# tum-vision/mem

Measured on AMD Instinct MI355X. Metric: pretrain samples/sec (ViT-B, 224^2 event voxels), higher is better.
Workload: dtype bf16; 1 GPU; MEM pretrain ViT-Base/16, 224^2 2-bin event voxels, bf16, batch 256 per GPU (BASELINE configs[1]); step = rasterize 256x30k events + event_norm + masks + ViT fwd/CE/bwd + clip + AdamW; global_batch=256, parallelism=dp1, stochastic_depth=work skipping, optimizer=AdamW as one launch in front of the next forward, last_block_mlp_rows=rows that reach the head

## Files before the change

### mem_amd/csrc/rowops.hip

```cpp
#include "common.h"
#include "dropout.hpp"

namespace {

using namespace memhip;

typedef __attribute__((ext_vector_type(4))) __bf16 bf16x4;
typedef __attribute__((ext_vector_type(8))) __bf16 bf16x8;

__device__ __forceinline__ float wsum(float v) {
  for (int o = 32; o > 0; o >>= 1) v += __shfl_xor(v, o);
  return v;
}
__device__ __forceinline__ float wmax(float v) {
  for (int o = 32; o > 0; o >>= 1) v = fmaxf(v, __shfl_xor(v, o));
  return v;
}

__device__ __forceinline__ float div_newton(float a, float b, float r) {
  const float q0 = a * r;
  return fmaf(fmaf(-q0, b, a), r, q0);
}

constexpr int kMaxChunks = 8;

__global__ __launch_bounds__(256) void ln_fwd_kernel(const float* __restrict__ x, long long ldx,
                                                     const int* __restrict__ row_idx, int R, int D,
                                                     const float* __restrict__ gamma,
                                                     const float* __restrict__ beta, float eps,
                                                     __bf16* __restrict__ y, long long ldy,
                                                     float* __restrict__ mean, float* __restrict__ rstd) {
  const int lane = threadIdx.x & 63;
  const int r = blockIdx.x * 4 + (threadIdx.x >> 6);
  if (r >= R) return;
  const long long src = row_idx ? row_idx[r] : r;
  const float4* xr = reinterpret_cast<const float4*>(x + src * ldx);
  const int nch = D >> 2;
  float4 v[kMaxChunks];
  float s = 0.f;
#pragma unroll
  for (int c = 0; c < kMaxChunks; ++c) {
    const int i = lane + c * 64;
    if (i < nch) { v[c] = xr[i]; s += (v[c].x + v[c].y) + (v[c].z + v[c].w); }
  }
  const float mu = wsum(s) / (float)D;
  float q = 0.f;
#pragma unroll
  for (int c = 0; c < kMaxChunks; ++c) {
    const int i = lane + c * 64;
    if (i < nch) {
      const float a = v[c].x - mu, b = v[c].y - mu, cc = v[c].z - mu, d = v[c].w - mu;
      q += (a * a + b * b) + (cc * cc + d * d);
    }
  }
  const float var = wsum(q) / (float)D;
  const float rs = 1.0f / sqrtf(var + eps);
  if (lane == 0) { mean[r] = mu; rstd[r] = rs; }
  const float4* g4 = reinterpret_cast<const float4*>(gamma);
  const float4* b4 = reinterpret_cast<const float4*>(beta);
  bf16x4* yr = reinterpret_cast<bf16x4*>(y + (long long)r * ldy);
#pragma unroll
  for (int c = 0; c < kMaxChunks; ++c) {
    const int i = lane + c * 64;
    if (i < nch) {
      const float4 g = g4[i], b = b4[i];
      bf16x4 o;
      o[0] = (__bf16)((v[c].x - mu) * rs * g.x + b.x);
      o[1] = (__bf16)((v[c].y - mu) * rs * g.y + b.y);
      o[2] = (__bf16)((v[c].z - mu) * rs * g.z + b.z);
      o[3] = (__bf16)((v[c].w - mu) * rs * g.w + b.w);
      yr[i] = o;
    }
  }
}


template <int NCH>
__global__ __launch_bounds__(256) void ln_bwd_kernel(const __bf16* __restrict__ dy, long long lddy,
                                                     const float* __restrict__ x, long long ldx,
                                                     const int* __restrict__ row_idx, int R, int D,
                                                     const float* __restrict__ gamma,
                                                     const float* __restrict__ mean,
                                                     const float* __restrict__ rstd,
                                                     float* __restrict__ dres, long long lddres,
                                                     int accumulate, float* __restrict__ dgamma,
                                                     float* __restrict__ dbeta) {
  extern __shared__ float red[];
  const int lane = threadIdx.x & 63, wave = threadIdx.x >> 6;
  const int nch = D >> 2;
  const float4* g4 = reinterpret_cast<const float4*>(gamma);
  float4 ag[NCH], ab[NCH], gm[NCH];
#pragma unroll
  for (int c = 0; c < NCH; ++c) {
    ag[c] = float4{0, 0, 0, 0};
    ab[c] = float4{0, 0, 0, 0};
    gm[c] = (lane + c * 64 < nch) ? g4[lane + c * 64] : float4{0, 0, 0, 0};
  }
  for (int r = blockIdx.x * 4 + wave; r < R; r += gridDim.x * 4) {
    const long long src = row_idx ? row_idx[r] : r;
    const float4* xr = reinterpret_cast<const float4*>(x + src * ldx);
    const bf16x4* dyr = reinterpret_cast<const bf16x4*>(dy + (long long)r * lddy);
    const float mu = mean[r], rs = rstd[r];
    float4 xh[NCH], gg[NCH], prev[NCH];
    float4* o = reinterpret_cast<float4*>(dres + src * lddres);
    if (accumulate) {
#pragma unroll
      for (int c = 0; c < NCH; ++c)
        if (lane + c * 64 < nch) prev[c] = o[lane + c * 64];
    }
    float s1 = 0.f, s2 = 0.f;
#pragma unroll
    for (int c = 0; c < NCH; ++c) {
      const int i = lane + c * 64;
      if (i < nch) {
        const float4 xv = xr[i];
        const bf16x4 d4 = dyr[i];
        const float4 g = gm[c];
        const float d0 = (float)d4[0], d1 = (float)d4[1], d2 = (float)d4[2], d3 = (float)d4[3];
        xh[c] = float4{(xv.x - mu) * rs, (xv.y - mu) * rs, (xv.z - mu) * rs, (xv.w - mu) * rs};
        gg[c] = float4{d0 * g.x, d1 * g.y, d2 * g.z, d3 * g.w};
        s1 += (gg[c].x + gg[c].y) + (gg[c].z + gg[c].w);
        s2 += (gg[c].x * xh[c].x + gg[c].y * xh[c].y) + (gg[c].z * xh[c].z + gg[c].w * xh[c].w);
        ag[c].x += d0 * xh[c].x; ag[c].y += d1 * xh[c].y; ag[c].z += d2 * xh[c].z; ag[c].w += d3 * xh[c].w;
        ab[c].x += d0; ab[c].y += d1; ab[c].z += d2; ab[c].w += d3;
      }
    }
    const float m1 = wsum(s1) / (float)D, m2 = wsum(s2) / (float)D;
#pragma unroll
    for (int c = 0; c < NCH; ++c) {
      const int i = lane + c * 64;
      if (i < nch) {
        float4 d{rs * (gg[c].x - m1 - xh[c].x * m2), rs * (gg[c].y - m1 - xh[c].y * m2),
                 rs * (gg[c].z - m1 - xh[c].z * m2), rs * (gg[c].w - m1 - xh[c].w * m2)};
        if (accumulate) { const float4 p = prev[c]; d.x += p.x; d.y += p.y; d.z += p.z; d.w += p.w; }
        o[i] = d;
      }
    }
  }
  float4* rg = reinterpret_cast<float4*>(red + (size_t)wave * 2 * D);
  float4* rb = reinterpret_cast<float4*>(red + (size_t)wave * 2 * D + D);
#pragma unroll
  for (int c = 0; c < NCH; ++c) {
    const int i = lane + c * 64;
    if (i < nch) { rg[i] = ag[c]; rb[i] = ab[c]; }
  }
  __syncthreads();
  for (int n = threadIdx.x; n < D; n += 256) {
    float a = 0.f, b = 0.f;
#pragma unroll
    for (int w = 0; w < 4; ++w) { a += red[(size_t)w * 2 * D + n]; b += red[(size_t)w * 2 * D + D + n]; }
    atomicAdd(dgamma + n, a);
    atomicAdd(dbeta + n, b);
  }
}

constexpr int kBrMaxChunks = 8;

template <int NCH, class... Drop>
__global__ __launch_bounds__(256) void branch_bwd_kernel(const float* __restrict__ dx, long long lddx,
                                                         const __bf16* __restrict__ y, long long ldy,
                                                         const float* __restrict__ gamma,
                                                         const float* __restrict__ rowmask, float keep,
                                                         int rps, int M, int D, __bf16* __restrict__ dyo,
                                                         long long lddy, float* __restrict__ dgamma,
                                                         float* __restrict__ dbias, const int* __restrict__ out_map,
                                                         Drop... drop) {
  extern __shared__ float red[];
  const int lane = threadIdx.x & 63, wave = threadIdx.x >> 6;
  const int nch = D >> 2;
  float4 g[NCH], ag[NCH], ab[NCH];
  const float rk = __frcp_rn(keep);
#pragma unroll
  for (int c = 0; c < NCH; ++c) {
    const int i = lane + c * 64;
    g[c] = (gamma && i < nch) ? reinterpret_cast<const float4*>(gamma)[i] : float4{1.f, 1.f, 1.f, 1.f};
    ag[c] = float4{0, 0, 0, 0};
    ab[c] = float4{0, 0, 0, 0};
  }
  const int stride = gridDim.x * 4;
  for (int m0 = blockIdx.x * 4 + wave; m0 < M; m0 += 2 * stride) {
    float4 dv[2][NCH];
    bf16x4 yv[2][NCH];
    float kk[2];
    long long mo[2];
#pragma unroll
    for (int u = 0; u < 2; ++u) {
      const int m = m0 + u * stride;
      const int mc = m < M ? m : M - 1;
      const float4* dr = reinterpret_cast<const float4*>(dx + (long long)mc * lddx);
      kk[u] = rowmask ? rowmask[mc / rps] : 1.f;
      mo[u] = m < M ? m : -1;
      if (out_map && m < M) {
        const int smp = mc / rps, co = out_map[smp];
        mo[u] = co < 0 ? -1 : (long long)co * rps + (mc - smp * rps);
      }
      if (mo[u] < 0) continue;
#pragma unroll
      for (int c = 0; c < NCH; ++c) {
        const int i = lane + c * 64;
        if (i < nch) {
          dv[u][c] = dr[i];
          if (y) yv[u][c] = reinterpret_cast<const bf16x4*>(y + (long long)mc * ldy)[i];
        }
      }
    }
#pragma unroll
    for (int u = 0; u < 2; ++u) {
      if (mo[u] < 0) continue;
      bf16x4* orow = reinterpret_cast<bf16x4*>(dyo + mo[u] * lddy);
      const float k = kk[u];
#pragma unroll
      for (int c = 0; c < NCH; ++c) {
        const int i = lane + c * 64;
        if (i < nch) {
          float4 d = dv[u][c];
          if (rowmask || out_map) {
            d.x = div_newton(d.x * k, keep, rk); d.y = div_newton(d.y * k, keep, rk);
            d.z = div_newton(d.z * k, keep, rk); d.w = div_newton(d.w * k, keep, rk);
          }
          if constexpr (sizeof...(Drop) > 0) {
            const DropParams dp = (drop, ...);
            const unsigned kb = dropout_keep8(dp, (unsigned)(dp.row0 + m0 + u * stride), (unsigned)(i >> 1)) >> ((i & 1) * 4);
            d.x = __fmul_rn(d.x, dropout_mul(dp, kb, 0)); d.y = __fmul_rn(d.y, dropout_mul(dp, kb, 1));
            d.z = __fmul_rn(d.z, dropout_mul(dp, kb, 2)); d.w = __fmul_rn(d.w, dropout_mul(dp, kb, 3));
          }
          if (y) {
            const bf16x4 yy = yv[u][c];
            ag[c].x += d.x * (float)yy[0]; ag[c].y += d.y * (float)yy[1];
            ag[c].z += d.z * (float)yy[2]; ag[c].w += d.w * (float)yy[3];
          }
          bf16x4 o;
          o[0] = (__bf16)(d.x * g[c].x); o[1] = (__bf16)(d.y * g[c].y);
          o[2] = (__bf16)(d.z * g[c].z); o[3] = (__bf16)(d.w * g[c].w);
          orow[i] = o;
          ab[c].x += (float)o[0]; ab[c].y += (float)o[1]; ab[c].z += (float)o[2]; ab[c].w += (float)o[3];
        }
      }
    }
  }
  float4* rg = reinterpret_cast<float4*>(red + (size_t)wave * 2 * D);
  float4* rb = reinterpret_cast<float4*>(red + (size_t)wave * 2 * D + D);
#pragma unroll
  for (int c = 0; c < NCH; ++c) {
    const int i = lane + c * 64;
    if (i < nch) { rg[i] = ag[c]; rb[i] = ab[c]; }
  }
  __syncthreads();
  for (int n = threadIdx.x; n < D; n += 256) {
    float a = 0.f, b = 0.f;
#pragma unroll
    for (int w = 0; w < 4; ++w) { a += red[(size_t)w * 2 * D + n]; b += red[(size_t)w * 2 * D + D + n]; }
    if (dgamma) atomicAdd(dgamma + n, a);
    if (dbias) atomicAdd(dbias + n, b);
  }
}

template <int NCH, bool HAS_Y, class... Drop>
__global__ __launch_bounds__(256) void ln_bwd_branch_kernel(const __bf16* __restrict__ dy, long long lddy,
                                                            const float* __restrict__ x, long long ldx, int R, int D,
                                                            const float* __restrict__ gamma,
                                                            const float* __restrict__ mean, const float* __restrict__ rstd,
                                                            float* __restrict__ dres, long long lddres,
                                                            float* __restrict__ dgamma, float* __restrict__ dbeta,
                                                            const __bf16* __restrict__ yb, long long ldyb,
                                                            const float* __restrict__ gb, const float* __restrict__ rowmask,
                                                            float keep, int rps, __bf16* __restrict__ dyo, long long lddyo,
                                                            float* __restrict__ dgb, float* __restrict__ dbiasb,
                                                            const int* __restrict__ in_map, const int* __restrict__ out_map,
                                                            Drop... drop) {
  extern __shared__ float red[];
  const int lane = threadIdx.x & 63, wave = threadIdx.x >> 6;
  const int nch = D >> 2;
  float4 ag[NCH], ab[NCH], bg[HAS_Y ? NCH : 1], bb[NCH];
  const float4* g4 = reinterpret_cast<const float4*>(gamma);
  const float4* gb4 = reinterpret_cast<const float4*>(gb);
  const float rk = __frcp_rn(keep);
#pragma unroll
  for (int c = 0; c < NCH; ++c) {
    ag[c] = ab[c] = bb[c] = float4{0, 0, 0, 0};
    if (HAS_Y) bg[c] = float4{0, 0, 0, 0};
  }
  const int rstride = gridDim.x * 4;
  float4 xn[NCH], pn[NCH];
  bf16x4 dn[NCH], yn[HAS_Y ? NCH : 1];
  long long rin_n = 0, rout_n = 0;
  auto load_row = [&](int r) {
    rin_n = r; rout_n = r;
    if (in_map || out_map) {
      const int smp = r / rps, off = r - smp * rps;
      if (in_map) { const int ci = in_map[smp]; rin_n = ci < 0 ? -1 : (long long)ci * rps + off; }
      if (out_map) { const int co = out_map[smp]; rout_n = co < 0 ? -1 : (long long)co * rps + off; }
    }
    if (rin_n < 0 && rout_n < 0) return;
    const float4* xr = reinterpret_cast<const float4*>(x + (long long)r * ldx);
    const bf16x4* dyr = reinterpret_cast<const bf16x4*>(dy + (rin_n < 0 ? 0 : rin_n) * lddy);
    const float4* o = reinterpret_cast<const float4*>(dres + (long long)r * lddres);
#pragma unroll
    for (int c = 0; c < NCH; ++c) {
      const int i = lane + c * 64;
      if (i < nch) {
        pn[c] = o[i];
        if (rin_n >= 0) {
          xn[c] = xr[i];
          dn[c] = dyr[i];
        }
        if constexpr (HAS_Y) yn[c] = reinterpret_cast<const bf16x4*>(yb + (long long)r * ldyb)[i];
      }
    }
  };
  int r = blockIdx.x * 4 + wave;
  if (r < R) load_row(r);
  for (; r < R; r += rstride) {
    const long long rin = rin_n, rout = rout_n;
    if (rin < 0 && rout < 0) {
      if (r + rstride < R) load_row(r + rstride);
      continue;
    }
    float4* o = reinterpret_cast<float4*>(dres + (long long)r * lddres);
    const float mu = rin >= 0 ? mean[rin] : 0.f, rs = rin >= 0 ? rstd[rin] : 0.f;
    const float km = rowmask ? rowmask[r / rps] : 1.f;
    float4 xh[NCH], gg[NCH], prev[NCH];
    bf16x4 yv[HAS_Y ? NCH : 1];
    float s1 = 0.f, s2 = 0.f;
#pragma unroll
    for (int c = 0; c < NCH; ++c) {
      const int i = lane + c * 64;
      if (i < nch) {
        prev[c] = pn[c];
        if constexpr (HAS_Y) yv[c] = yn[c];
        if (rin < 0) {
          xh[c] = gg[c] = float4{0.f, 0.f, 0.f, 0.f};
          continue;
        }
        const float4 xv = xn[c];
        const bf16x4 d4 = dn[c];
        const float d0 = (float)d4[0], d1 = (float)d4[1], d2 = (float)d4[2], d3 = (float)d4[3];
        xh[c] = float4{(xv.x - mu) * rs, (xv.y - mu) * rs, (xv.z - mu) * rs, (xv.w - mu) * rs};
        const float4 gmc = g4[i];
        gg[c] = float4{d0 * gmc.x, d1 * gmc.y, d2 * gmc.z, d3 * gmc.w};
        s1 += (gg[c].x + gg[c].y) + (gg[c].z + gg[c].w);
        s2 += (gg[c].x * xh[c].x + gg[c].y * xh[c].y) + (gg[c].z * xh[c].z + gg[c].w * xh[c].w);
        ag[c].x += d0 * xh[c].x; ag[c].y += d1 * xh[c].y; ag[c].z += d2 * xh[c].z; ag[c].w += d3 * xh[c].w;
        ab[c].x += d0; ab[c].y += d1; ab[c].z += d2; ab[c].w += d3;
      }
    }
    if (r + rstride < R) load_row(r + rstride);
    const float m1 = wsum(s1) / (float)D, m2 = wsum(s2) / (float)D;
    bf16x4* orow = reinterpret_cast<bf16x4*>(dyo + (rout < 0 ? 0 : rout) * lddyo);
#pragma unroll
    for (int c = 0; c < NCH; ++c) {
      const int i = lane + c * 64;
      if (i < nch) {
        float4 d{prev[c].x + rs * (gg[c].x - m1 - xh[c].x * m2), prev[c].y + rs * (gg[c].y - m1 - xh[c].y * m2),
                 prev[c].z + rs * (gg[c].z - m1 - xh[c].z * m2), prev[c].w + rs * (gg[c].w - m1 - xh[c].w * m2)};
        if (rin >= 0) o[i] = d;
        if (rout < 0) continue;
        if (rowmask || out_map) {
          d.x = div_newton(d.x * km, keep, rk); d.y = div_newton(d.y * km, keep, rk);
          d.z = div_newton(d.z * km, keep, rk); d.w = div_newton(d.w * km, keep, rk);
        }
        if constexpr (sizeof...(Drop) > 0) {
          const DropParams dp = (drop, ...);
          const unsigned kb = dropout_keep8(dp, (unsigned)(dp.row0 + r), (unsigned)(i >> 1)) >> ((i & 1) * 4);
          d.x = __fmul_rn(d.x, dropout_mul(dp, kb, 0)); d.y = __fmul_rn(d.y, dropout_mul(dp, kb, 1));
          d.z = __fmul_rn(d.z, dropout_mul(dp, kb, 2)); d.w = __fmul_rn(d.w, dropout_mul(dp, kb, 3));
        }
        if constexpr (HAS_Y) {
          bg[c].x += d.x * (float)yv[c][0]; bg[c].y += d.y * (float)yv[c][1];
          bg[c].z += d.z * (float)yv[c][2]; bg[c].w += d.w * (float)yv[c][3];
        }
        const float4 gbc = gb ? gb4[i] : float4{1.f, 1.f, 1.f, 1.f};
        bf16x4 q;
        q[0] = (__bf16)(d.x * gbc.x); q[1] = (__bf16)(d.y * gbc.y);
        q[2] = (__bf16)(d.z * gbc.z); q[3] = (__bf16)(d.w * gbc.w);
        orow[i] = q;
        bb[c].x += (float)q[0]; bb[c].y += (float)q[1]; bb[c].z += (float)q[2]; bb[c].w += (float)q[3];
      }
    }
  }
  float4* r0 = reinterpret_cast<float4*>(red + (size_t)wave * 4 * D);
#pragma unroll
  for (int c = 0; c < NCH; ++c) {
    const int i = lane + c * 64;
    if (i < nch) { r0[i] = ag[c]; r0[nch + i] = ab[c]; r0[2 * nch + i] = HAS_Y ? bg[HAS_Y ? c : 0] : float4{0, 0, 0, 0}; r0[3 * nch + i] = bb[c]; }
  }
  __syncthreads();
  for (int n = threadIdx.x; n < D; n += 256) {
    float a = 0.f, b = 0.f, c2 = 0.f, d2 = 0.f;
#pragma unroll
    for (int w = 0; w < 4; ++w) {
      const float* rw = red + (size_t)w * 4 * D;
      a += rw[n]; b += rw[D + n]; c2 += rw[2 * D + n]; d2 += rw[3 * D + n];
    }
    atomicAdd(dgamma + n, a);
    atomicAdd(dbeta + n, b);
    if (dgb) atomicAdd(dgb + n, c2);
    if (dbiasb) atomicAdd(dbiasb + n, d2);
  }
}


__global__ __launch_bounds__(256) void layerscale_grad_kernel(const __bf16* __restrict__ W, long long ldw,
                                                              const float* __restrict__ dW, long long lddw,
                                                              const float* __restrict__ b, const float* __restrict__ db,
                                                              const float* __restrict__ gamma, int N, int K,
                                                              float* __restrict__ dgamma) {
  __shared__ float red[4][4];
  const int lane = threadIdx.x & 63, wave = threadIdx.x >> 6;
  const int n0 = blockIdx.x * 4;
  float s[4] = {0.f, 0.f, 0.f, 0.f};
  for (int k0 = 0; k0 < K; k0 += 4096) {
#pragma unroll
    for (int c = 0; c < 4; ++c) {
      const int n = n0 + c < N ? n0 + c : N - 1;
      const __bf16* wr = W + (long long)n * ldw;
      const float* gr = dW + (long long)n * lddw;
#pragma unroll
      for (int u = 0; u < 4; ++u) {
        const int k = k0 + u * 1024 + (int)threadIdx.x * 4;
        if (k < K) {
          const bf16x4 w = *reinterpret_cast<const bf16x4*>(wr + k);
          const float4 g = *reinterpret_cast<const float4*>(gr + k);
          s[c] += (float)w[0] * g.x + (float)w[1] * g.y + (float)w[2] * g.z + (float)w[3] * g.w;
        }
      }
    }
  }
#pragma unroll
  for (int c = 0; c < 4; ++c) {
    const float t = wsum(s[c]);
    if (lane == 0) red[wave][c] = t;
  }
  __syncthreads();
  if (threadIdx.x < 4 && n0 + (int)threadIdx.x < N) {
    const int n = n0 + threadIdx.x;
    float t = (red[0][threadIdx.x] + red[1][threadIdx.x]) + (red[2][threadIdx.x] + red[3][threadIdx.x]);
    if (b && db) t += b[n] * db[n];
    const float g = gamma[n];
    dgamma[n] = g != 0.f ? t / g : 0.f;
  }
}

__global__ __launch_bounds__(256) void embed_bwd_kernel(const float* __restrict__ dx, long long lddx,
                                                        const unsigned char* __restrict__ mask, int B,
                                                        int L, int D, __bf16* __restrict__ dy,
                                                        long long lddy, float* __restrict__ dcls,
                                                        float* __restrict__ dmask) {
  constexpr int U = 7;
  for (int c = threadIdx.x * 4; c < D; c += 256 * 4) {
    float4 cls{0, 0, 0, 0}, am{0, 0, 0, 0};
    for (int b = blockIdx.x; b < B; b += gridDim.x) {
      const float* row0 = dx + (long long)b * (L + 1) * lddx + c;
      const float4 dc = *reinterpret_cast<const float4*>(row0);
      cls.x += dc.x; cls.y += dc.y; cls.z += dc.z; cls.w += dc.w;
      const unsigned char* mk = mask + (long long)b * L;
      __bf16* out = dy + (long long)b * L * lddy + c;
      int p = 0;
      for (; p + U <= L; p += U) {
        float4 d[U];
#pragma unroll
        for (int u = 0; u < U; ++u) d[u] = *reinterpret_cast<const float4*>(row0 + (long long)(1 + p + u) * lddx);
#pragma unroll
        for (int u = 0; u < U; ++u) {
          const float w = (float)mk[p + u], q = 1.0f - w;
          am.x += d[u].x * w; am.y += d[u].y * w; am.z += d[u].z * w; am.w += d[u].w * w;
          bf16x4 o;
          o[0] = (__bf16)(d[u].x * q); o[1] = (__bf16)(d[u].y * q); o[2] = (__bf16)(d[u].z * q); o[3] = (__bf16)(d[u].w * q);
          *reinterpret_cast<bf16x4*>(out + (long long)(p + u) * lddy) = o;
        }
      }
      for (; p < L; ++p) {
        const float4 d = *reinterpret_cast<const float4*>(row0 + (long long)(1 + p) * lddx);
        const float w = (float)mk[p], q = 1.0f - w;
        am.x += d.x * w; am.y += d.y * w; am.z += d.z * w; am.w += d.w * w;
        bf16x4 o;
        o[0] = (__bf16)(d.x * q); o[1] = (__bf16)(d.y * q); o[2] = (__bf16)(d.z * q); o[3] = (__bf16)(d.w * q);
        *reinterpret_cast<bf16x4*>(out + (long long)p * lddy) = o;
      }
    }
    atomicAdd(dcls + c, cls.x); atomicAdd(dcls + c + 1, cls.y);
    atomicAdd(dcls + c + 2, cls.z); atomicAdd(dcls + c + 3, cls.w);
    atomicAdd(dmask + c, am.x); atomicAdd(dmask + c + 1, am.y);
    atomicAdd(dmask + c + 2, am.z); atomicAdd(dmask + c + 3, am.w);
  }
}

template <int VPT>
__global__ __launch_bounds__(256) void ce_kernel(__bf16* __restrict__ logits, long long ld,
                                                 const long long* __restrict__ labels, int V,
                                                 float grad_scale, float* __restrict__ row_loss,
                                                 int* __restrict__ row_correct, int write_grad) {
  __shared__ float sm[4];
  __shared__ int si[4];
  __shared__ float bc[2];
  const int r = blockIdx.x, tid = threadIdx.x, lane = tid & 63, wave = tid >> 6;
  bf16x8* row = reinterpret_cast<bf16x8*>(logits + (long long)r * ld);
  const int nch = V >> 3;
  float v[VPT][8];
  float mx = -INFINITY;
  int amax = 0x7fffffff;
#pragma unroll
  for (int c = 0; c < VPT; ++c) {
    const int i = tid + c * 256;
    if (i < nch) {
      const bf16x8 t = row[i];
#pragma unroll
      for (int k = 0; k < 8; ++k) {
        v[c][k] = (float)t[k];
        if (v[c][k] > mx) { mx = v[c][k]; amax = i * 8 + k; }
      }
    }
  }
  for (int o = 32; o > 0; o >>= 1) {
    const float om = __shfl_xor(mx, o);
    const int oi = __shfl_xor(amax, o);
    if (om > mx || (om == mx && oi < amax)) { mx = om; amax = oi; }
  }
  if (lane == 0) { sm[wave] = mx; si[wave] = amax; }
  __syncthreads();
  if (tid == 0) {
    float m = sm[0]; int a = si[0];
    for (int w = 1; w < 4; ++w) if (sm[w] > m || (sm[w] == m && si[w] < a)) { m = sm[w]; a = si[w]; }
    bc[0] = m; si[0] = a;
  }
  __syncthreads();
  mx = bc[0];
  amax = si[0];
  float s = 0.f;
#pragma unroll
  for (int c = 0; c < VPT; ++c) {
    const int i = tid + c * 256;
    if (i < nch) {
#pragma unroll
      for (int k = 0; k < 8; ++k) { v[c][k] = __expf(v[c][k] - mx); s += v[c][k]; }
    }
  }
  s = wsum(s);
  __syncthreads();
  if (lane == 0) sm[wave] = s;
  __syncthreads();
  if (tid == 0) bc[1] = (sm[0] + sm[1]) + (sm[2] + sm[3]);
  __syncthreads();
  const float sum = bc[1];
  const long long lab = labels[r];
  if (tid == 0) {
    const bool lab_ok = lab >= 0 && lab < V;
    const float zl = lab_ok ? (float)logits[(long long)r * ld + lab] : __builtin_nanf("");
    row_loss[r] = (mx + __logf(sum)) - zl;
    row_correct[r] = (amax == (int)lab) ? 1 : 0;
  }
  if (write_grad) {
    const float inv = 1.0f / sum;
    __syncthreads();
#pragma unroll
    for (int c = 0; c < VPT; ++c) {
      const int i = tid + c * 256;
      if (i < nch) {
        bf16x8 o;
#pragma unroll
        for (int k = 0; k < 8; ++k) {
          float p = v[c][k] * inv;
          if ((long long)(i * 8 + k) == lab) p -= 1.0f;
          o[k] = (__bf16)(p * grad_scale);
        }
        row[i] = o;
      }
    }
  }
}

__global__ __launch_bounds__(256) void ce_reduce_kernel(const float* __restrict__ row_loss,
                                                        const int* __restrict__ row_correct, int M,
                                                        float* __restrict__ out) {
  __shared__ double sd[4];
  __shared__ int sc[4];
  double s = 0.0;
  int c = 0;
  for (int i = threadIdx.x; i < M; i += 256) { s += (double)row_loss[i]; c += row_correct[i]; }
  for (int o = 32; o > 0; o >>= 1) { s += __shfl_xor(s, o); c += __shfl_xor(c, o); }
  if ((threadIdx.x & 63) == 0) { sd[threadIdx.x >> 6] = s; sc[threadIdx.x >> 6] = c; }
  __syncthreads();
  if (threadIdx.x == 0) {
    const double t = (sd[0] + sd[1]) + (sd[2] + sd[3]);
    const int k = sc[0] + sc[1] + sc[2] + sc[3];
    out[0] = (float)(t / (double)M);
    out[1] = (float)k / (float)M;
  }
}

}

extern "C" int memhip_layernorm_fwd(const float* x, int64_t ldx, const int32_t* row_idx, int R, int D,
                                    const float* gamma, const float* beta, float eps, void* y,
                                    int64_t ldy, float* mean, float* rstd, memhip_stream_t stream) {
  MEMHIP_REQUIRE(R >= 0 && D > 0 && D % 4 == 0 && D <= 64 * 4 * kMaxChunks, "layernorm_fwd: bad R=%d D=%d", R, D);
  if (R == 0) return MEMHIP_OK;
  MEMHIP_REQUIRE(x && gamma && beta && y && mean && rstd, "layernorm_fwd: null pointer");
  MEMHIP_REQUIRE(ldx % 4 == 0 && ldy % 4 == 0, "layernorm_fwd: ld must be a multiple of 4");
  hipLaunchKernelGGL(ln_fwd_kernel, dim3(cdiv(R, 4)), dim3(256), 0, as_stream(stream), x, (long long)ldx,
                     row_idx, R, D, gamma, beta, eps, (__bf16*)y, (long long)ldy, mean, rstd);
  return check_launch("layernorm_fwd");
}

extern "C" int memhip_layernorm_bwd(const void* dy, int64_t lddy, const float* x, int64_t ldx,
                                    const int32_t* row_idx, int R, int D, const float* gamma,
                                    const float* mean, const float* rstd, float* dres, int64_t lddres,
                                    int accumulate, float* dgamma, float* dbeta, memhip_stream_t stream) {
  MEMHIP_REQUIRE(R >= 0 && D > 0 && D % 4 == 0 && D <= 64 * 4 * kMaxChunks, "layernorm_bwd: bad R=%d D=%d", R, D);
  if (R == 0) return MEMHIP_OK;
  MEMHIP_REQUIRE(dy && x && gamma && mean && rstd && dres && dgamma && dbeta, "layernorm_bwd: null pointer");
  MEMHIP_REQUIRE(ldx % 4 == 0 && lddy % 4 == 0 && lddres % 4 == 0, "layernorm_bwd: ld must be a multiple of 4");
  int grid = cdiv(R, 4);
  const int cap = opt(OPT_LN_BWD_GRID) * 4 / 3;
  if (grid > cap) grid = cap;
#define LNB_LAUNCH(N)                                                                                    \
  hipLaunchKernelGGL(ln_bwd_kernel<N>, dim3(grid), dim3(256), (size_t)8 * D * sizeof(float), as_stream(stream), \
                     (const __bf16*)dy, (long long)lddy, x, (long long)ldx, row_idx, R, D, gamma, mean, rstd, dres, \
                     (long long)lddres, accumulate, dgamma, dbeta)
  const int nchl = cdiv(D / 4, 64);
  if (nchl <= 1) LNB_LAUNCH(1);
  else if (nchl <= 2) LNB_LAUNCH(2);
  else if (nchl <= 3) LNB_LAUNCH(3);
  else if (nchl <= 4) LNB_LAUNCH(4);
  else LNB_LAUNCH(8);
#undef LNB_LAUNCH
  return check_launch("layernorm_bwd");
}

static int branch_bwd_impl(const float* dx, int64_t lddx, const void* y, int64_t ldy,
                           const float* gamma, const float* rowmask, float keep_prob,
                           int rows_per_sample, int M, int D, void* dy, int64_t lddy,
                           float* dgamma, float* dbias, const int32_t* out_map, const memhip_dropout_t* drop,
                           memhip_stream_t stream) {
  MEMHIP_REQUIRE(M >= 0 && D > 0 && D % 4 == 0, "branch_bwd: bad M=%d D=%d", M, D);
  MEMHIP_REQUIRE(!drop || D % 8 == 0, "branch_bwd_drop: D=%d must be a multiple of 8", D);
  MEMHIP_REQUIRE(!out_map || (!rowmask && !y && rows_per_sample > 0), "branch_bwd: out_map excludes rowmask / y");
  if (M == 0) return MEMHIP_OK;
  MEMHIP_REQUIRE(dx && dy, "branch_bwd: null pointer");
  MEMHIP_REQUIRE(y || !dgamma, "branch_bwd: dgamma needs y (or use memhip_layerscale_grad)");
  MEMHIP_REQUIRE(lddx % 4 == 0 && ldy % 4 == 0 && lddy % 4 == 0, "branch_bwd: ld must be a multiple of 4");
  MEMHIP_REQUIRE(D <= 64 * 4 * kBrMaxChunks, "branch_bwd: D=%d too large", D);
  int grid = cdiv(M, 4);
  if (grid > 1024) grid = 1024;
#define BRB_LAUNCH(N)                                                                                    \
  if (drop) BRB_LAUNCH_D(N); else                                                                        \
  hipLaunchKernelGGL(branch_bwd_kernel<N>, dim3(grid), dim3(256), (size_t)8 * D * sizeof(float), as_stream(stream), \
                     dx, (long long)lddx, (const __bf16*)y, (long long)ldy, gamma, rowmask, keep_prob,    \
                     rows_per_sample > 0 ? rows_per_sample : 1, M, D, (__bf16*)dy, (long long)lddy, dgamma, dbias, \
                     (const int*)out_map)
#define BRB_LAUNCH_D(N)                                                                                  \
  hipLaunchKernelGGL((branch_bwd_kernel<N, DropParams>), dim3(grid), dim3(256), (size_t)8 * D * sizeof(float),  \
                     as_stream(stream), dx, (long long)lddx, (const __bf16*)y, (long long)ldy, gamma, rowmask, keep_prob, \
                     rows_per_sample > 0 ? rows_per_sample : 1, M, D, (__bf16*)dy, (long long)lddy, dgamma, dbias, \
                     (const int*)out_map, drop_params(*drop))
  const int nchl = cdiv(D / 4, 64);
  if (nchl <= 1) BRB_LAUNCH(1);
  else if (nchl <= 2) BRB_LAUNCH(2);
  else if (nchl <= 3) BRB_LAUNCH(3);
  else if (nchl <= 4) BRB_LAUNCH(4);
  else BRB_LAUNCH(8);
#undef BRB_LAUNCH
#undef BRB_LAUNCH_D
  return check_launch("branch_bwd");
}

extern "C" int memhip_branch_bwd_map(const float* dx, int64_t lddx, const void* y, int64_t ldy,
                                     const float* gamma, const float* rowmask, float keep_prob,
                                     int rows_per_sample, int M, int D, void* dy, int64_t lddy,
                                     float* dgamma, float* dbias, const int32_t* out_map, memhip_stream_t stream) {
  return branch_bwd_impl(dx, lddx, y, ldy, gamma, rowmask, keep_prob, rows_per_sample, M, D, dy, lddy, dgamma, dbias, out_map,
                         nullptr, stream);
}

extern "C" int memhip_branch_bwd_drop(const float* dx, int64_t lddx, const void* y, int64_t ldy,
                                      const float* gamma, const float* rowmask, float keep_prob,
                                      int rows_per_sample, int M, int D, void* dy, int64_t lddy,
                                      float* dgamma, float* dbias, const int32_t* out_map, const memhip_dropout_t* dropout,
                                      memhip_stream_t stream) {
  MEMHIP_REQUIRE(dropout, "branch_bwd_drop: null dropout");
  return branch_bwd_impl(dx, lddx, y, ldy, gamma, rowmask, keep_prob, rows_per_sample, M, D, dy, lddy, dgamma, dbias, out_map,
                         dropout, stream);
}

extern "C" int memhip_branch_bwd(const float* dx, int64_t lddx, const void* y, int64_t ldy,
                                 const float* gamma, const float* rowmask, float keep_prob,
                                 int rows_per_sample, int M, int D, void* dy, int64_t lddy,
                                 float* dgamma, float* dbias, memhip_stream_t stream) {
  return memhip_branch_bwd_map(dx, lddx, y, ldy, gamma, rowmask, keep_prob, rows_per_sample, M, D, dy, lddy, dgamma, dbias,
                               nullptr, stream);
}

extern "C" int memhip_embed_bwd(const float* dx, int64_t lddx, const uint8_t* mask, int B, int L, int D,
                                void* dy, int64_t lddy, float* dcls, float* dmask_token,
                                memhip_stream_t stream) {
  MEMHIP_REQUIRE(B >= 0 && L > 0 && D > 0 && D % 4 == 0, "embed_bwd: bad shape");
  if (B == 0) return MEMHIP_OK;
  MEMHIP_REQUIRE(dx && mask && dy && dcls && dmask_token, "embed_bwd: null pointer");
  hipLaunchKernelGGL(embed_bwd_kernel, dim3(B < 128 ? B : 128), dim3(256), 0, as_stream(stream), dx, (long long)lddx, mask, B,
                     L, D, (__bf16*)dy, (long long)lddy, dcls, dmask_token);
  return check_launch("embed_bwd");
}

extern "C" int memhip_cross_entropy(void* logits, int64_t ld, const int64_t* labels, int M, int V,
                                    float grad_scale, float* row_loss, int32_t* row_correct,
                                    int write_grad, float* out2, memhip_stream_t stream) {
  MEMHIP_REQUIRE(M >= 0 && V > 0 && V % 8 == 0 && V <= 256 * 8 * 8, "cross_entropy: V=%d unsupported", V);
  if (M == 0) return MEMHIP_OK;
  MEMHIP_REQUIRE(logits && labels && row_loss && row_correct && out2, "cross_entropy: null pointer");
  MEMHIP_REQUIRE(ld % 8 == 0, "cross_entropy: ld must be a multiple of 8");
  hipStream_t s = as_stream(stream);
  const int nch = V / 8, vpt = cdiv(nch, 256);
  __bf16* lg = (__bf16*)logits;
  const long long* lab = (const long long*)labels;
#define CE_LAUNCH(N) hipLaunchKernelGGL(ce_kernel<N>, dim3(M), dim3(256), 0, s, lg, (long long)ld, lab, V, \
                                        grad_scale, row_loss, row_correct, write_grad)
  if (vpt <= 1) CE_LAUNCH(1);
  else if (vpt <= 2) CE_LAUNCH(2);
  else if (vpt <= 4) CE_LAUNCH(4);
  else CE_LAUNCH(8);
#undef CE_LAUNCH
  hipLaunchKernelGGL(ce_reduce_kernel, dim3(1), dim3(256), 0, s, row_loss, row_correct, M, out2);
  return check_launch("cross_entropy");
}

static int ln_bwd_branch_impl(const void* dy, int64_t lddy, const float* x, int64_t ldx, int R, int D,
                              const float* gamma, const float* mean, const float* rstd, float* dres,
                              int64_t lddres, float* dgamma, float* dbeta, const void* y_branch,
                              int64_t ldyb, const float* gamma_branch, const float* rowmask,
                              float keep_prob, int rows_per_sample, void* dy_branch, int64_t lddyb,
                              float* dgamma_branch, float* dbias_branch, const int32_t* in_map,
                              const int32_t* out_map, const memhip_dropout_t* drop, memhip_stream_t stream) {
  MEMHIP_REQUIRE(R >= 0 && D > 0 && D % 4 == 0 && D <= 64 * 4 * 4, "layernorm_bwd_branch: D=%d unsupported (<= 1024)", D);
  MEMHIP_REQUIRE(!drop || D % 8 == 0, "layernorm_bwd_branch_drop: D=%d must be a multiple of 8", D);
  MEMHIP_REQUIRE(!(in_map || out_map) || (!rowmask && !y_branch && rows_per_sample > 0),
                 "layernorm_bwd_branch: sample maps exclude rowmask / y_branch");
  if (R == 0) return MEMHIP_OK;
  MEMHIP_REQUIRE(dy && x && gamma && mean && rstd && dres && dgamma && dbeta && dy_branch,
                 "layernorm_bwd_branch: null pointer");
  MEMHIP_REQUIRE(y_branch || !dgamma_branch, "layernorm_bwd_branch: dgamma_branch needs y_branch");
  MEMHIP_REQUIRE(ldx % 4 == 0 && lddy % 4 == 0 && lddres % 4 == 0 && ldyb % 4 == 0 && lddyb % 4 == 0,
                 "layernorm_bwd_branch: ld must be a multiple of 4");
  int grid = cdiv(R, 4);
  int cap = opt(OPT_LN_BWD_GRID);
  if (D > 768 && cap > 512) cap = 512;
  if (grid > cap) grid = cap;
#define LBB_LAUNCH(N)                                                                                    \
  if (drop) { if (y_branch) LBB_LAUNCH2D(N, true); else LBB_LAUNCH2D(N, false); }                       \
  else if (y_branch) LBB_LAUNCH2(N, true); else LBB_LAUNCH2(N, false)
#define LBB_LAUNCH2(N, Y)                                                                                \
  hipLaunchKernelGGL((ln_bwd_branch_kernel<N, Y>), dim3(grid), dim3(256), (size_t)16 * D * sizeof(float), \
                     as_stream(stream), (const __bf16*)dy, (long long)lddy, x, (long long)ldx, R, D, gamma, mean, \
                     rstd, dres, (long long)lddres, dgamma, dbeta, (const __bf16*)y_branch, (long long)ldyb, \
                     gamma_branch, rowmask, keep_prob, rows_per_sample > 0 ? rows_per_sample : 1,         \
                     (__bf16*)dy_branch, (long long)lddyb, dgamma_branch, dbias_branch, (const int*)in_map, \
                     (const int*)out_map)
#define LBB_LAUNCH2D(N, Y)                                                                               \
  hipLaunchKernelGGL((ln_bwd_branch_kernel<N, Y, DropParams>), dim3(grid), dim3(256), (size_t)16 * D * sizeof(float), \
                     as_stream(stream), (const __bf16*)dy, (long long)lddy, x, (long long)ldx, R, D, gamma, mean, \
                     rstd, dres, (long long)lddres, dgamma, dbeta, (const __bf16*)y_branch, (long long)ldyb, \
                     gamma_branch, rowmask, keep_prob, rows_per_sample > 0 ? rows_per_sample : 1,         \
                     (__bf16*)dy_branch, (long long)lddyb, dgamma_branch, dbias_branch, (const int*)in_map, \
                     (const int*)out_map, drop_params(*drop))
  const int nchl = cdiv(D / 4, 64);
  if (nchl <= 1) LBB_LAUNCH(1);
  else if (nchl <= 2) LBB_LAUNCH(2);
  else if (nchl <= 3) LBB_LAUNCH(3);
  else LBB_LAUNCH(4);
#undef LBB_LAUNCH
#undef LBB_LAUNCH2
#undef LBB_LAUNCH2D
  return check_launch("layernorm_bwd_branch");
}

extern "C" int memhip_layernorm_bwd_branch_map(const void* dy, int64_t lddy, const float* x, int64_t ldx, int R, int D,
                                               const float* gamma, const float* mean, const float* rstd, float* dres,
                                               int64_t lddres, float* dgamma, float* dbeta, const void* y_branch,
                                               int64_t ldyb, const float* gamma_branch, const float* rowmask,
                                               float keep_prob, int rows_per_sample, void* dy_branch, int64_t lddyb,
                                               float* dgamma_branch, float* dbias_branch, const int32_t* in_map,
                                               const int32_t* out_map, memhip_stream_t stream) {
  return ln_bwd_branch_impl(dy, lddy, x, ldx, R, D, gamma, mean, rstd, dres, lddres, dgamma, dbeta, y_branch, ldyb,
                            gamma_branch, rowmask, keep_prob, rows_per_sample, dy_branch, lddyb, dgamma_branch, dbias_branch,
                            in_map, out_map, nullptr, stream);
}

extern "C" int memhip_layernorm_bwd_branch_drop(const void* dy, int64_t lddy, const float* x, int64_t ldx, int R, int D,
                                                const float* gamma, const float* mean, const float* rstd, float* dres,
                                                int64_t lddres, float* dgamma, float* dbeta, const void* y_branch,
                                                int64_t ldyb, const float* gamma_branch, const float* rowmask,
                                                float keep_prob, int rows_per_sample, void* dy_branch, int64_t lddyb,
                                                float* dgamma_branch, float* dbias_branch, const int32_t* in_map,
                                                const int32_t* out_map, const memhip_dropout_t* dropout,
                                                memhip_stream_t stream) {
  MEMHIP_REQUIRE(dropout, "layernorm_bwd_branch_drop: null dropout");
  return ln_bwd_branch_impl(dy, lddy, x, ldx, R, D, gamma, mean, rstd, dres, lddres, dgamma, dbeta, y_branch, ldyb,
                            gamma_branch, rowmask, keep_prob, rows_per_sample, dy_branch, lddyb, dgamma_branch, dbias_branch,
                            in_map, out_map, dropout, stream);
}

extern "C" int memhip_layernorm_bwd_branch(const void* dy, int64_t lddy, const float* x, int64_t ldx, int R, int D,
                                           const float* gamma, const float* mean, const float* rstd, float* dres,
                                           int64_t lddres, float* dgamma, float* dbeta, const void* y_branch,
                                           int64_t ldyb, const float* gamma_branch, const float* rowmask,
                                           float keep_prob, int rows_per_sample, void* dy_branch, int64_t lddyb,
                                           float* dgamma_branch, float* dbias_branch, memhip_stream_t stream) {
  return memhip_layernorm_bwd_branch_map(dy, lddy, x, ldx, R, D, gamma, mean, rstd, dres, lddres, dgamma, dbeta, y_branch,
                                         ldyb, gamma_branch, rowmask, keep_prob, rows_per_sample, dy_branch, lddyb,
                                         dgamma_branch, dbias_branch, nullptr, nullptr, stream);
}

extern "C" int memhip_layerscale_grad(const void* W_bf16, int64_t ldw, const float* dW, int64_t lddw, const float* bias,
                                      const float* dbias, const float* gamma, int N, int K, float* dgamma,
                                      memhip_stream_t stream) {
  MEMHIP_REQUIRE(N >= 0 && K > 0 && K % 4 == 0 && ldw % 4 == 0 && lddw % 4 == 0, "layerscale_grad: bad shape");
  if (N == 0) return MEMHIP_OK;
  MEMHIP_REQUIRE(W_bf16 && dW && gamma && dgamma && (!bias == !dbias), "layerscale_grad: null pointer");
  hipLaunchKernelGGL(layerscale_grad_kernel, dim3((N + 3) / 4), dim3(256), 0, as_stream(stream), (const __bf16*)W_bf16,
                     (long long)ldw, dW, (long long)lddw, bias, dbias, gamma, N, K, dgamma);
  return check_launch("layerscale_grad");
}
```

Before: 7520 samples/sec.

## Software-pipeline LayerNorm and branch backward row kernels with templated full-chunk variants

Reworks the row-wise LayerNorm forward/backward and branch-backward kernels. Loads for the next row are issued before the current row is reduced and written, so memory latency overlaps with compute. Gamma/beta are staged in shared memory instead of held in registers. Chunk bounds checks and the accumulate/has-y flags become template parameters, and fp contraction is pinned to keep rounding stable. This adds register pressure and template instantiations, and a hand-written waitcnt drain may be fragile.

```diff
diff --git a/mem_amd/csrc/rowops.hip b/mem_amd/csrc/rowops.hip
--- a/mem_amd/csrc/rowops.hip
+++ b/mem_amd/csrc/rowops.hip
@@ -1,5 +1,7 @@
 #include "common.h"
 #include "dropout.hpp"
+
+#include <type_traits>
 
 namespace {
 
@@ -24,58 +26,124 @@
 
 constexpr int kMaxChunks = 8;
 
+template <bool FULL>
+__device__ __forceinline__ bool chunk_ok(int i, int nch) {
+  if constexpr (FULL) return true;
+  else return i < nch;
+}
+
+__device__ __forceinline__ int wave_id() { return __builtin_amdgcn_readfirstlane((int)(threadIdx.x >> 6)); }
+
+struct RowWalk {
+  int r, smp, off, stride, q, rem, rps;
+  __device__ __forceinline__ RowWalk(int r0, int stride_, int rps_) : r(r0), stride(stride_), rps(rps_) {
+    smp = r0 / rps; off = r0 - smp * rps;
+    q = stride / rps; rem = stride - q * rps;
+  }
+  __device__ __forceinline__ void next() {
+    r += stride; smp += q; off += rem;
+    if (off >= rps) { off -= rps; ++smp; }
+  }
+};
+
+__device__ __forceinline__ void stage_columns(float4* dst, const float* a, const float* b, int nch) {
+  for (int i = threadIdx.x; i < nch; i += 256) {
+    dst[i] = reinterpret_cast<const float4*>(a)[i];
+    dst[nch + i] = b ? reinterpret_cast<const float4*>(b)[i] : float4{1.f, 1.f, 1.f, 1.f};
+  }
+  __syncthreads();
+}
+
+__device__ __forceinline__ int opaque(int v) {
+  asm volatile("" : "+v"(v));
+  return v;
+}
+
+__device__ __forceinline__ float mul_rn(float a, float b) {
+#pragma clang fp contract(off)
+  return a * b;
+}
+__device__ __forceinline__ float sub_rn(float a, float b) {
+#pragma clang fp contract(off)
+  return a - b;
+}
+__device__ __forceinline__ float ln_dx(float gg, float xh, float m1, float m2) { return __fmaf_rn(-xh, m2, sub_rn(gg, m1)); }
+__device__ __forceinline__ float sq2(float a, float b) { return __fmaf_rn(a, a, mul_rn(b, b)); }
+
+template <int NCH, bool FULL>
 __global__ __launch_bounds__(256) void ln_fwd_kernel(const float* __restrict__ x, long long ldx,
                                                      const int* __restrict__ row_idx, int R, int D,
                                                      const float* __restrict__ gamma,
                                                      const float* __restrict__ beta, float eps,
                                                      __bf16* __restrict__ y, long long ldy,
                                                      float* __restrict__ mean, float* __restrict__ rstd) {
+  extern __shared__ float red[];
   const int lane = threadIdx.x & 63;
-  const int r = blockIdx.x * 4 + (threadIdx.x >> 6);
-  if (r >= R) return;
+  const int r0 = blockIdx.x * 4 + wave_id();
+  const bool act = r0 < R;
+  const int r = act ? r0 : R - 1;
   const long long src = row_idx ? row_idx[r] : r;
   const float4* xr = reinterpret_cast<const float4*>(x + src * ldx);
   const int nch = D >> 2;
-  float4 v[kMaxChunks];
+  float4 v[NCH];
+#pragma unroll
+  for (int c = 0; c < NCH; ++c) {
+    const int i = lane + c * 64;
+    if (chunk_ok<FULL>(i, nch)) v[c] = xr[i];
+  }
+  constexpr int NST = (64 * NCH + 255) / 256;
+  float4 sg[NST], sb[NST];
+#pragma unroll
+  for (int k = 0; k < NST; ++k) {
+    const int i = min((int)threadIdx.x + k * 256, nch - 1);
+    sg[k] = reinterpret_cast<const float4*>(gamma)[i];
+    sb[k] = reinterpret_cast<const float4*>(beta)[i];
+  }
+  __builtin_amdgcn_sched_barrier(0);
   float s = 0.f;
 #pragma unroll
-  for (int c = 0; c < kMaxChunks; ++c) {
-    const int i = lane + c * 64;
-    if (i < nch) { v[c] = xr[i]; s += (v[c].x + v[c].y) + (v[c].z + v[c].w); }
-  }
+  for (int c = 0; c < NCH; ++c)
+    if (chunk_ok<FULL>(lane + c * 64, nch)) s += (v[c].x + v[c].y) + (v[c].z + v[c].w);
   const float mu = wsum(s) / (float)D;
+  float4* lgb = reinterpret_cast<float4*>(red);
+#pragma unroll
+  for (int k = 0; k < NST; ++k) {
+    const int i = min((int)threadIdx.x + k * 256, nch - 1);
+    lgb[i] = sg[k];
+    lgb[nch + i] = sb[k];
+  }
   float q = 0.f;
 #pragma unroll
-  for (int c = 0; c < kMaxChunks; ++c) {
-    const int i = lane + c * 64;
-    if (i < nch) {
+  for (int c = 0; c < NCH; ++c) {
+    if (chunk_ok<FULL>(lane + c * 64, nch)) {
       const float a = v[c].x - mu, b = v[c].y - mu, cc = v[c].z - mu, d = v[c].w - mu;
-      q += (a * a + b * b) + (cc * cc + d * d);
+      q += sq2(a, b) + sq2(cc, d);
     }
   }
   const float var = wsum(q) / (float)D;
   const float rs = 1.0f / sqrtf(var + eps);
+  __syncthreads();
+  if (!act) return;
   if (lane == 0) { mean[r] = mu; rstd[r] = rs; }
-  const float4* g4 = reinterpret_cast<const float4*>(gamma);
-  const float4* b4 = reinterpret_cast<const float4*>(beta);
   bf16x4* yr = reinterpret_cast<bf16x4*>(y + (long long)r * ldy);
 #pragma unroll
-  for (int c = 0; c < kMaxChunks; ++c) {
+  for (int c = 0; c < NCH; ++c) {
     const int i = lane + c * 64;
-    if (i < nch) {
-      const float4 g = g4[i], b = b4[i];
+    if (chunk_ok<FULL>(i, nch)) {
+      const float4 g = lgb[i], b = lgb[nch + i];
       bf16x4 o;
-      o[0] = (__bf16)((v[c].x - mu) * rs * g.x + b.x);
-      o[1] = (__bf16)((v[c].y - mu) * rs * g.y + b.y);
-      o[2] = (__bf16)((v[c].z - mu) * rs * g.z + b.z);
-      o[3] = (__bf16)((v[c].w - mu) * rs * g.w + b.w);
+      o[0] = (__bf16)__fmaf_rn(mul_rn(v[c].x - mu, rs), g.x, b.x);
+      o[1] = (__bf16)__fmaf_rn(mul_rn(v[c].y - mu, rs), g.y, b.y);
+      o[2] = (__bf16)__fmaf_rn(mul_rn(v[c].z - mu, rs), g.z, b.z);
+      o[3] = (__bf16)__fmaf_rn(mul_rn(v[c].w - mu, rs), g.w, b.w);
       yr[i] = o;
     }
   }
 }
 
-
-template <int NCH>
+__device__ __forceinline__ void vm_drain() { __builtin_amdgcn_s_waitcnt(0x0F70); }
+
+template <int NCH, bool FULL, bool ACC>
 __global__ __launch_bounds__(256) void ln_bwd_kernel(const __bf16* __restrict__ dy, long long lddy,
                                                      const float* __restrict__ x, long long ldx,
                                                      const int* __restrict__ row_idx, int R, int D,
@@ -83,66 +151,120 @@
                                                      const float* __restrict__ mean,
                                                      const float* __restrict__ rstd,
                                                      float* __restrict__ dres, long long lddres,
-                                                     int accumulate, float* __restrict__ dgamma,
-                                                     float* __restrict__ dbeta) {
+                                                     float* __restrict__ dgamma, float* __restrict__ dbeta) {
   extern __shared__ float red[];
-  const int lane = threadIdx.x & 63, wave = threadIdx.x >> 6;
+  const int lane = threadIdx.x & 63, wave = wave_id();
   const int nch = D >> 2;
-  const float4* g4 = reinterpret_cast<const float4*>(gamma);
-  float4 ag[NCH], ab[NCH], gm[NCH];
+  float4 ag[NCH], ab[NCH];
 #pragma unroll
   for (int c = 0; c < NCH; ++c) {
     ag[c] = float4{0, 0, 0, 0};
     ab[c] = float4{0, 0, 0, 0};
-    gm[c] = (lane + c * 64 < nch) ? g4[lane + c * 64] : float4{0, 0, 0, 0};
-  }
-  for (int r = blockIdx.x * 4 + wave; r < R; r += gridDim.x * 4) {
-    const long long src = row_idx ? row_idx[r] : r;
+  }
+  const int rstride = gridDim.x * 4;
+  float4 xn[NCH], prev[NCH];
+  bf16x4 dn[NCH];
+  auto issue = [&](int r, long long src, int lane) {
     const float4* xr = reinterpret_cast<const float4*>(x + src * ldx);
     const bf16x4* dyr = reinterpret_cast<const bf16x4*>(dy + (long long)r * lddy);
-    const float mu = mean[r], rs = rstd[r];
-    float4 xh[NCH], gg[NCH], prev[NCH];
-    float4* o = reinterpret_cast<float4*>(dres + src * lddres);
-    if (accumulate) {
-#pragma unroll
-      for (int c = 0; c < NCH; ++c)
-        if (lane + c * 64 < nch) prev[c] = o[lane + c * 64];
-    }
-    float s1 = 0.f, s2 = 0.f;
 #pragma unroll
     for (int c = 0; c < NCH; ++c) {
       const int i = lane + c * 64;
-      if (i < nch) {
-        const float4 xv = xr[i];
-        const bf16x4 d4 = dyr[i];
-        const float4 g = gm[c];
+      if (chunk_ok<FULL>(i, nch)) {
+        xn[c] = xr[i];
+        dn[c] = dyr[i];
+      }
+    }
+  };
+  auto issue_prev = [&](long long src, int lane) {
+    const float4* o = reinterpret_cast<const float4*>(dres + src * lddres);
+#pragma unroll
+    for (int c = 0; c < NCH; ++c) {
+      const int i = lane + c * 64;
+      if (chunk_ok<FULL>(i, nch)) prev[c] = o[i];
+    }
+  };
+  int r = blockIdx.x * 4 + wave;
+  long long src = 0;
+  float mu = 0.f, rs = 0.f;
+  if (r < R) {
+    src = row_idx ? row_idx[r] : r;
+    issue(r, src, lane);
+    if constexpr (ACC) issue_prev(src, lane);
+    mu = mean[r]; rs = rstd[r];
+  }
+  float4* lg = reinterpret_cast<float4*>(red);
+  for (int i = threadIdx.x; i < nch; i += 256) lg[i] = reinterpret_cast<const float4*>(gamma)[i];
+  __syncthreads();
+  int r1 = r + rstride;
+  long long src1 = 0;
+  if (r1 < R) src1 = row_idx ? row_idx[r1] : r1;
+  int r2 = r1 + rstride;
+  vm_drain();
+  while (r < R) {
+    float4 xh[NCH], gg[NCH];
+    float s1 = 0.f, s2 = 0.f;
+    const int ol = opaque(lane);
+    const float4* lgl = lg + ol;
+#pragma unroll
+    for (int c = 0; c < NCH; ++c) {
+      const int i = lane + c * 64;
+      if (chunk_ok<FULL>(i, nch)) {
+        const float4 xv = xn[c];
+        const bf16x4 d4 = dn[c];
+        const float4 g = lgl[c * 64];
         const float d0 = (float)d4[0], d1 = (float)d4[1], d2 = (float)d4[2], d3 = (float)d4[3];
-        xh[c] = float4{(xv.x - mu) * rs, (xv.y - mu) * rs, (xv.z - mu) * rs, (xv.w - mu) * rs};
-        gg[c] = float4{d0 * g.x, d1 * g.y, d2 * g.z, d3 * g.w};
+        xh[c] = float4{mul_rn(xv.x - mu, rs), mul_rn(xv.y - mu, rs), mul_rn(xv.z - mu, rs), mul_rn(xv.w - mu, rs)};
+        gg[c] = float4{mul_rn(d0, g.x), mul_rn(d1, g.y), mul_rn(d2, g.z), mul_rn(d3, g.w)};
         s1 += (gg[c].x + gg[c].y) + (gg[c].z + gg[c].w);
-        s2 += (gg[c].x * xh[c].x + gg[c].y * xh[c].y) + (gg[c].z * xh[c].z + gg[c].w * xh[c].w);
+        s2 += (mul_rn(gg[c].x, xh[c].x) + mul_rn(gg[c].y, xh[c].y)) + (mul_rn(gg[c].z, xh[c].z) + mul_rn(gg[c].w, xh[c].w));
         ag[c].x += d0 * xh[c].x; ag[c].y += d1 * xh[c].y; ag[c].z += d2 * xh[c].z; ag[c].w += d3 * xh[c].w;
         ab[c].x += d0; ab[c].y += d1; ab[c].z += d2; ab[c].w += d3;
       }
     }
+    float mu1 = 0.f, rs1 = 0.f;
+    long long src2 = 0;
+    const bool next = r1 < R;
+    const int rl = next ? r1 : r;
+    const long long srcl = next ? src1 : src;
+    issue(rl, srcl, ol);
+    if (next) {
+      mu1 = mean[r1]; rs1 = rstd[r1];
+      if (r2 < R) src2 = row_idx ? row_idx[r2] : r2;
+    }
     const float m1 = wsum(s1) / (float)D, m2 = wsum(s2) / (float)D;
+    float4* o = reinterpret_cast<float4*>(dres + src * lddres);
 #pragma unroll
     for (int c = 0; c < NCH; ++c) {
-      const int i = lane + c * 64;
-      if (i < nch) {
-        float4 d{rs * (gg[c].x - m1 - xh[c].x * m2), rs * (gg[c].y - m1 - xh[c].y * m2),
-                 rs * (gg[c].z - m1 - xh[c].z * m2), rs * (gg[c].w - m1 - xh[c].w * m2)};
-        if (accumulate) { const float4 p = prev[c]; d.x += p.x; d.y += p.y; d.z += p.z; d.w += p.w; }
+      const int i = ol + c * 64;
+      if (chunk_ok<FULL>(i, nch)) {
+        const float4 t{ln_dx(gg[c].x, xh[c].x, m1, m2), ln_dx(gg[c].y, xh[c].y, m1, m2),
+                       ln_dx(gg[c].z, xh[c].z, m1, m2), ln_dx(gg[c].w, xh[c].w, m1, m2)};
+        float4 d;
+        if constexpr (ACC) {
+          const float4 p = prev[c];
+          d = float4{__fmaf_rn(rs, t.x, p.x), __fmaf_rn(rs, t.y, p.y), __fmaf_rn(rs, t.z, p.z), __fmaf_rn(rs, t.w, p.w)};
+        } else {
+          d = float4{mul_rn(rs, t.x), mul_rn(rs, t.y), mul_rn(rs, t.z), mul_rn(rs, t.w)};
+        }
         o[i] = d;
       }
     }
-  }
+    if constexpr (ACC) {
+      __builtin_amdgcn_sched_barrier(0);
+      issue_prev(srcl, ol);
+    }
+    r = r1; src = src1; mu = mu1; rs = rs1;
+    r1 = r2; src1 = src2;
+    r2 += rstride;
+  }
+  __syncthreads();
   float4* rg = reinterpret_cast<float4*>(red + (size_t)wave * 2 * D);
   float4* rb = reinterpret_cast<float4*>(red + (size_t)wave * 2 * D + D);
 #pragma unroll
   for (int c = 0; c < NCH; ++c) {
     const int i = lane + c * 64;
-    if (i < nch) { rg[i] = ag[c]; rb[i] = ab[c]; }
+    if (chunk_ok<FULL>(i, nch)) { rg[i] = ag[c]; rb[i] = ab[c]; }
   }
   __syncthreads();
   for (int n = threadIdx.x; n < D; n += 256) {
@@ -156,7 +278,7 @@
 
 constexpr int kBrMaxChunks = 8;
 
-template <int NCH, class... Drop>
+template <int NCH, bool FULL, bool HAS_Y, class... Drop>
 __global__ __launch_bounds__(256) void branch_bwd_kernel(const float* __restrict__ dx, long long lddx,
                                                          const __bf16* __restrict__ y, long long ldy,
                                                          const float* __restrict__ gamma,
@@ -166,96 +288,122 @@
                                                          float* __restrict__ dbias, const int* __restrict__ out_map,
                                                          Drop... drop) {
   extern __shared__ float red[];
-  const int lane = threadIdx.x & 63, wave = threadIdx.x >> 6;
+  const int lane = threadIdx.x & 63, wave = wave_id();
   const int nch = D >> 2;
-  float4 g[NCH], ag[NCH], ab[NCH];
+  float4 ag[NCH], ab[NCH];
   const float rk = __frcp_rn(keep);
+#pragma unroll
+  for (int c = 0; c < NCH; ++c) {
+    ag[c] = float4{0, 0, 0, 0};
+    ab[c] = float4{0, 0, 0, 0};
+  }
+  float4 dn[NCH];
+  bf16x4 yn[HAS_Y ? NCH : 1];
+  auto issue = [&](int m, int lane) {
+    const float4* dr = reinterpret_cast<const float4*>(dx + (long long)m * lddx);
+#pragma unroll
+    for (int c = 0; c < NCH; ++c) {
+      const int i = lane + c * 64;
+      if (chunk_ok<FULL>(i, nch)) {
+        dn[c] = dr[i];
+        if constexpr (HAS_Y) yn[c] = reinterpret_cast<const bf16x4*>(y + (long long)m * ldy)[i];
+      }
+    }
+  };
+  RowWalk w(blockIdx.x * 4 + wave, gridDim.x * 4, rps);
+  auto find = [&](int& m, int& mo, int& smp) {
+    for (;;) {
+      m = w.r; smp = w.smp; mo = -1;
+      if (m >= M) return;
+      mo = w.r;
+      if (out_map) { const int co = out_map[w.smp]; mo = co < 0 ? -1 : co * w.rps + w.off; }
+      w.next();
+      if (mo >= 0) return;
+    }
+  };
+  int m, mo, smp;
+  float k = 1.f;
+  find(m, mo, smp);
+  if (m < M) {
+    issue(m, lane);
+    if (rowmask) k = rowmask[smp];
+  }
+  float4* lg = reinterpret_cast<float4*>(red);
+  for (int i = threadIdx.x; i < nch; i += 256)
+    lg[i] = gamma ? reinterpret_cast<const float4*>(gamma)[i] : float4{1.f, 1.f, 1.f, 1.f};
+  __syncthreads();
+  int m1, mo1, smp1;
+  find(m1, mo1, smp1);
+  vm_drain();
+  while (m < M) {
+    const int ol = opaque(lane);
+    float4 dv[NCH];
+    bf16x4 yv[HAS_Y ? NCH : 1];
+#pragma unroll
+    for (int c = 0; c < NCH; ++c) {
+      if (chunk_ok<FULL>(lane + c * 64, nch)) {
+        dv[c] = dn[c];
+        if constexpr (HAS_Y) yv[c] = yn[c];
+      }
+    }
+    float k1 = 1.f;
+    const bool next = m1 < M;
+    issue(next ? m1 : m, ol);
+    if (next && rowmask) k1 = rowmask[smp1];
+    int m2, mo2, smp2;
+    find(m2, mo2, smp2);
+    bf16x4* orow = reinterpret_cast<bf16x4*>(dyo + (long long)mo * lddy);
+    const float4* lgl = lg + ol;
+#pragma unroll
+    for (int c = 0; c < NCH; ++c) {
+      const int i = ol + c * 64;
+      if (chunk_ok<FULL>(i, nch)) {
+        float4 d = dv[c];
+        if (rowmask || out_map) {
+          d.x = div_newton(d.x * k, keep, rk); d.y = div_newton(d.y * k, keep, rk);
+          d.z = div_newton(d.z * k, keep, rk); d.w = div_newton(d.w * k, keep, rk);
+        }
+        if constexpr (sizeof...(Drop) > 0) {
+          const DropParams dp = (drop, ...);
+          const unsigned kb = dropout_keep8(dp, (unsigned)(dp.row0 + m), (unsigned)(i >> 1)) >> ((i & 1) * 4);
+          d.x = __fmul_rn(d.x, dropout_mul(dp, kb, 0)); d.y = __fmul_rn(d.y, dropout_mul(dp, kb, 1));
+          d.z = __fmul_rn(d.z, dropout_mul(dp, kb, 2)); d.w = __fmul_rn(d.w, dropout_mul(dp, kb, 3));
+        }
+        if constexpr (HAS_Y) {
+          const bf16x4 yy = yv[c];
+          ag[c].x += d.x * (float)yy[0]; ag[c].y += d.y * (float)yy[1];
+          ag[c].z += d.z * (float)yy[2]; ag[c].w += d.w * (float)yy[3];
+        }
+        const float4 g = lgl[c * 64];
+        bf16x4 o;
+        o[0] = (__bf16)(d.x * g.x); o[1] = (__bf16)(d.y * g.y);
+        o[2] = (__bf16)(d.z * g.z); o[3] = (__bf16)(d.w * g.w);
+        orow[i] = o;
+        ab[c].x += (float)o[0]; ab[c].y += (float)o[1]; ab[c].z += (float)o[2]; ab[c].w += (float)o[3];
+      }
+    }
+    m = m1; mo = mo1; k = k1;
+    m1 = m2; mo1 = mo2; smp1 = smp2;
+  }
+  __syncthreads();
+  float4* rg = reinterpret_cast<float4*>(red + (size_t)wave * 2 * D);
+  float4* rb = reinterpret_cast<float4*>(red + (size_t)wave * 2 * D + D);
 #pragma unroll
   for (int c = 0; c < NCH; ++c) {
     const int i = lane + c * 64;
-    g[c] = (gamma && i < nch) ? reinterpret_cast<const float4*>(gamma)[i] : float4{1.f, 1.f, 1.f, 1.f};
-    ag[c] = float4{0, 0, 0, 0};
-    ab[c] = float4{0, 0, 0, 0};
-  }
-  const int stride = gridDim.x * 4;
-  for (int m0 = blockIdx.x * 4 + wave; m0 < M; m0 += 2 * stride) {
-    float4 dv[2][NCH];
-    bf16x4 yv[2][NCH];
-    float kk[2];
-    long long mo[2];
-#pragma unroll
-    for (int u = 0; u < 2; ++u) {
-      const int m = m0 + u * stride;
-      const int mc = m < M ? m : M - 1;
-      const float4* dr = reinterpret_cast<const float4*>(dx + (long long)mc * lddx);
-      kk[u] = rowmask ? rowmask[mc / rps] : 1.f;
-      mo[u] = m < M ? m : -1;
-      if (out_map && m < M) {
-        const int smp = mc / rps, co = out_map[smp];
-        mo[u] = co < 0 ? -1 : (long long)co * rps + (mc - smp * rps);
-      }
-      if (mo[u] < 0) continue;
-#pragma unroll
-      for (int c = 0; c < NCH; ++c) {
-        const int i = lane + c * 64;
-        if (i < nch) {
-          dv[u][c] = dr[i];
-          if (y) yv[u][c] = reinterpret_cast<const bf16x4*>(y + (long long)mc * ldy)[i];
-        }
-      }
-    }
-#pragma unroll
-    for (int u = 0; u < 2; ++u) {
-      if (mo[u] < 0) continue;
-      bf16x4* orow = reinterpret_cast<bf16x4*>(dyo + mo[u] * lddy);
-      const float k = kk[u];
-#pragma unroll
-      for (int c = 0; c < NCH; ++c) {
-        const int i = lane + c * 64;
-        if (i < nch) {
-          float4 d = dv[u][c];
-          if (rowmask || out_map) {
-            d.x = div_newton(d.x * k, keep, rk); d.y = div_newton(d.y * k, keep, rk);
-            d.z = div_newton(d.z * k, keep, rk); d.w = div_newton(d.w * k, keep, rk);
-          }
-          if constexpr (sizeof...(Drop) > 0) {
-            const DropParams dp = (drop, ...);
-            const unsigned kb = dropout_keep8(dp, (unsigned)(dp.row0 + m0 + u * stride), (unsigned)(i >> 1)) >> ((i & 1) * 4);
-            d.x = __fmul_rn(d.x, dropout_mul(dp, kb, 0)); d.y = __fmul_rn(d.y, dropout_mul(dp, kb, 1));
-            d.z = __fmul_rn(d.z, dropout_mul(dp, kb, 2)); d.w = __fmul_rn(d.w, dropout_mul(dp, kb, 3));
-          }
-          if (y) {
-            const bf16x4 yy = yv[u][c];
-            ag[c].x += d.x * (float)yy[0]; ag[c].y += d.y * (float)yy[1];
-            ag[c].z += d.z * (float)yy[2]; ag[c].w += d.w * (float)yy[3];
-          }
-          bf16x4 o;
-          o[0] = (__bf16)(d.x * g[c].x); o[1] = (__bf16)(d.y * g[c].y);
-          o[2] = (__bf16)(d.z * g[c].z); o[3] = (__bf16)(d.w * g[c].w);
-          orow[i] = o;
-          ab[c].x += (float)o[0]; ab[c].y += (float)o[1]; ab[c].z += (float)o[2]; ab[c].w += (float)o[3];
-        }
-      }
-    }
-  }
-  float4* rg = reinterpret_cast<float4*>(red + (size_t)wave * 2 * D);
-  float4* rb = reinterpret_cast<float4*>(red + (size_t)wave * 2 * D + D);
-#pragma unroll
-  for (int c = 0; c < NCH; ++c) {
-    const int i = lane + c * 64;
-    if (i < nch) { rg[i] = ag[c]; rb[i] = ab[c]; }
+    if (chunk_ok<FULL>(i, nch)) { rg[i] = ag[c]; rb[i] = ab[c]; }
   }
   __syncthreads();
   for (int n = threadIdx.x; n < D; n += 256) {
     float a = 0.f, b = 0.f;
 #pragma unroll
-    for (int w = 0; w < 4; ++w) { a += red[(size_t)w * 2 * D + n]; b += red[(size_t)w * 2 * D + D + n]; }
+    for (int w2 = 0; w2 < 4; ++w2) { a += red[(size_t)w2 * 2 * D + n]; b += red[(size_t)w2 * 2 * D + D + n]; }
     if (dgamma) atomicAdd(dgamma + n, a);
     if (dbias) atomicAdd(dbias + n, b);
   }
 }
 
-template <int NCH, bool HAS_Y, class... Drop>
+template <int NCH, bool FULL, bool HAS_Y, class... Drop>
 __global__ __launch_bounds__(256) void ln_bwd_branch_kernel(const __bf16* __restrict__ dy, long long lddy,
                                                             const float* __restrict__ x, long long ldx, int R, int D,
                                                             const float* __restrict__ gamma,
@@ -269,92 +417,101 @@
                                                             const int* __restrict__ in_map, const int* __restrict__ out_map,
                                                             Drop... drop) {
   extern __shared__ float red[];
-  const int lane = threadIdx.x & 63, wave = threadIdx.x >> 6;
+  const int lane = threadIdx.x & 63, wave = wave_id();
   const int nch = D >> 2;
   float4 ag[NCH], ab[NCH], bg[HAS_Y ? NCH : 1], bb[NCH];
-  const float4* g4 = reinterpret_cast<const float4*>(gamma);
-  const float4* gb4 = reinterpret_cast<const float4*>(gb);
   const float rk = __frcp_rn(keep);
 #pragma unroll
   for (int c = 0; c < NCH; ++c) {
     ag[c] = ab[c] = bb[c] = float4{0, 0, 0, 0};
     if (HAS_Y) bg[c] = float4{0, 0, 0, 0};
   }
-  const int rstride = gridDim.x * 4;
-  float4 xn[NCH], pn[NCH];
+  float4 xn[NCH], prev[NCH];
   bf16x4 dn[NCH], yn[HAS_Y ? NCH : 1];
-  long long rin_n = 0, rout_n = 0;
-  auto load_row = [&](int r) {
-    rin_n = r; rout_n = r;
-    if (in_map || out_map) {
-      const int smp = r / rps, off = r - smp * rps;
-      if (in_map) { const int ci = in_map[smp]; rin_n = ci < 0 ? -1 : (long long)ci * rps + off; }
-      if (out_map) { const int co = out_map[smp]; rout_n = co < 0 ? -1 : (long long)co * rps + off; }
-    }
-    if (rin_n < 0 && rout_n < 0) return;
+  auto issue_x = [&](int r, int rin, int lane) {
     const float4* xr = reinterpret_cast<const float4*>(x + (long long)r * ldx);
-    const bf16x4* dyr = reinterpret_cast<const bf16x4*>(dy + (rin_n < 0 ? 0 : rin_n) * lddy);
-    const float4* o = reinterpret_cast<const float4*>(dres + (long long)r * lddres);
+    const bf16x4* dyr = reinterpret_cast<const bf16x4*>(dy + (long long)rin * lddy);
 #pragma unroll
     for (int c = 0; c < NCH; ++c) {
       const int i = lane + c * 64;
-      if (i < nch) {
-        pn[c] = o[i];
-        if (rin_n >= 0) {
-          xn[c] = xr[i];
-          dn[c] = dyr[i];
-        }
-        if constexpr (HAS_Y) yn[c] = reinterpret_cast<const bf16x4*>(yb + (long long)r * ldyb)[i];
+      if (chunk_ok<FULL>(i, nch)) {
+        xn[c] = xr[i];
+        dn[c] = dyr[i];
       }
     }
   };
-  int r = blockIdx.x * 4 + wave;
-  if (r < R) load_row(r);
-  for (; r < R; r += rstride) {
-    const long long rin = rin_n, rout = rout_n;
-    if (rin < 0 && rout < 0) {
-      if (r + rstride < R) load_row(r + rstride);
-      continue;
-    }
-    float4* o = reinterpret_cast<float4*>(dres + (long long)r * lddres);
-    const float mu = rin >= 0 ? mean[rin] : 0.f, rs = rin >= 0 ? rstd[rin] : 0.f;
-    const float km = rowmask ? rowmask[r / rps] : 1.f;
-    float4 xh[NCH], gg[NCH], prev[NCH];
-    bf16x4 yv[HAS_Y ? NCH : 1];
-    float s1 = 0.f, s2 = 0.f;
+  auto issue_y = [&](int r, int lane) {
+    if constexpr (HAS_Y) {
+#pragma unroll
+      for (int c = 0; c < NCH; ++c) {
+        const int i = lane + c * 64;
+        if (chunk_ok<FULL>(i, nch)) yn[c] = reinterpret_cast<const bf16x4*>(yb + (long long)r * ldyb)[i];
+      }
+    }
+  };
+  auto issue_prev = [&](int r, int lane) {
+    const float4* o = reinterpret_cast<const float4*>(dres + (long long)r * lddres);
 #pragma unroll
     for (int c = 0; c < NCH; ++c) {
       const int i = lane + c * 64;
-      if (i < nch) {
-        prev[c] = pn[c];
-        if constexpr (HAS_Y) yv[c] = yn[c];
-        if (rin < 0) {
+      if (chunk_ok<FULL>(i, nch)) prev[c] = o[i];
+    }
+  };
+  const int row0 = blockIdx.x * 4 + wave, rstride = gridDim.x * 4;
+  auto resolve = [&](const RowWalk& t, int& rin, int& rout) {
+    rin = rout = t.r;
+    if (in_map) { const int ci = in_map[t.smp]; rin = ci < 0 ? -1 : ci * t.rps + t.off; }
+    if (out_map) { const int co = out_map[t.smp]; rout = co < 0 ? -1 : co * t.rps + t.off; }
+  };
+  int r, rin, rout;
+  float mu = 0.f, rs = 0.f, km = 1.f;
+  float4 xh[NCH], gg[NCH];
+  bf16x4 yv[HAS_Y ? NCH : 1];
+  float s1, s2;
+  float4 *lg = reinterpret_cast<float4*>(red), *lgb = lg + nch;
+  auto reduce_row = [&](bool has_in, int ol) {
+    s1 = s2 = 0.f;
+    const float4* lgl = lg + ol;
+    if (has_in) {
+#pragma unroll
+      for (int c = 0; c < NCH; ++c) {
+        if (chunk_ok<FULL>(lane + c * 64, nch)) {
+          if constexpr (HAS_Y) yv[c] = yn[c];
+          const float4 xv = xn[c];
+          const bf16x4 d4 = dn[c];
+          const float d0 = (float)d4[0], d1 = (float)d4[1], d2 = (float)d4[2], d3 = (float)d4[3];
+          xh[c] = float4{mul_rn(xv.x - mu, rs), mul_rn(xv.y - mu, rs), mul_rn(xv.z - mu, rs), mul_rn(xv.w - mu, rs)};
+          const float4 gmc = lgl[c * 64];
+          gg[c] = float4{mul_rn(d0, gmc.x), mul_rn(d1, gmc.y), mul_rn(d2, gmc.z), mul_rn(d3, gmc.w)};
+          s1 += (gg[c].x + gg[c].y) + (gg[c].z + gg[c].w);
+          s2 += (mul_rn(gg[c].x, xh[c].x) + mul_rn(gg[c].y, xh[c].y)) + (mul_rn(gg[c].z, xh[c].z) + mul_rn(gg[c].w, xh[c].w));
+          ag[c].x += d0 * xh[c].x; ag[c].y += d1 * xh[c].y; ag[c].z += d2 * xh[c].z; ag[c].w += d3 * xh[c].w;
+          ab[c].x += d0; ab[c].y += d1; ab[c].z += d2; ab[c].w += d3;
+        }
+      }
+    } else {
+#pragma unroll
+      for (int c = 0; c < NCH; ++c) {
+        if (chunk_ok<FULL>(lane + c * 64, nch)) {
+          if constexpr (HAS_Y) yv[c] = yn[c];
           xh[c] = gg[c] = float4{0.f, 0.f, 0.f, 0.f};
-          continue;
-        }
-        const float4 xv = xn[c];
-        const bf16x4 d4 = dn[c];
-        const float d0 = (float)d4[0], d1 = (float)d4[1], d2 = (float)d4[2], d3 = (float)d4[3];
-        xh[c] = float4{(xv.x - mu) * rs, (xv.y - mu) * rs, (xv.z - mu) * rs, (xv.w - mu) * rs};
-        const float4 gmc = g4[i];
-        gg[c] = float4{d0 * gmc.x, d1 * gmc.y, d2 * gmc.z, d3 * gmc.w};
-        s1 += (gg[c].x + gg[c].y) + (gg[c].z + gg[c].w);
-        s2 += (gg[c].x * xh[c].x + gg[c].y * xh[c].y) + (gg[c].z * xh[c].z + gg[c].w * xh[c].w);
-        ag[c].x += d0 * xh[c].x; ag[c].y += d1 * xh[c].y; ag[c].z += d2 * xh[c].z; ag[c].w += d3 * xh[c].w;
-        ab[c].x += d0; ab[c].y += d1; ab[c].z += d2; ab[c].w += d3;
-      }
-    }
-    if (r + rstride < R) load_row(r + rstride);
+        }
+      }
+    }
+  };
+  auto store_row = [&](bool has_in, bool has_out, int ol) {
     const float m1 = wsum(s1) / (float)D, m2 = wsum(s2) / (float)D;
-    bf16x4* orow = reinterpret_cast<bf16x4*>(dyo + (rout < 0 ? 0 : rout) * lddyo);
+    float4* o = reinterpret_cast<float4*>(dres + (long long)r * lddres);
+    bf16x4* orow = reinterpret_cast<bf16x4*>(dyo + (long long)(has_out ? rout : 0) * lddyo);
+    const float4* lgbl = lgb + ol;
 #pragma unroll
     for (int c = 0; c < NCH; ++c) {
-      const int i = lane + c * 64;
-      if (i < nch) {
-        float4 d{prev[c].x + rs * (gg[c].x - m1 - xh[c].x * m2), prev[c].y + rs * (gg[c].y - m1 - xh[c].y * m2),
-                 prev[c].z + rs * (gg[c].z - m1 - xh[c].z * m2), prev[c].w + rs * (gg[c].w - m1 - xh[c].w * m2)};
-        if (rin >= 0) o[i] = d;
-        if (rout < 0) continue;
+      const int i = ol + c * 64;
+      if (chunk_ok<FULL>(i, nch)) {
+        float4 d{__fmaf_rn(rs, ln_dx(gg[c].x, xh[c].x, m1, m2), prev[c].x), __fmaf_rn(rs, ln_dx(gg[c].y, xh[c].y, m1, m2), prev[c].y),
+                 __fmaf_rn(rs, ln_dx(gg[c].z, xh[c].z, m1, m2), prev[c].z), __fmaf_rn(rs, ln_dx(gg[c].w, xh[c].w, m1, m2), prev[c].w)};
+        if (has_in) o[i] = d;
+        if (!has_out) continue;
         if (rowmask || out_map) {
           d.x = div_newton(d.x * km, keep, rk); d.y = div_newton(d.y * km, keep, rk);
           d.z = div_newton(d.z * km, keep, rk); d.w = div_newton(d.w * km, keep, rk);
@@ -369,7 +526,7 @@
           bg[c].x += d.x * (float)yv[c][0]; bg[c].y += d.y * (float)yv[c][1];
           bg[c].z += d.z * (float)yv[c][2]; bg[c].w += d.w * (float)yv[c][3];
         }
-        const float4 gbc = gb ? gb4[i] : float4{1.f, 1.f, 1.f, 1.f};
+        const float4 gbc = lgbl[c * 64];
         bf16x4 q;
         q[0] = (__bf16)(d.x * gbc.x); q[1] = (__bf16)(d.y * gbc.y);
         q[2] = (__bf16)(d.z * gbc.z); q[3] = (__bf16)(d.w * gbc.w);
@@ -377,19 +534,77 @@
         bb[c].x += (float)q[0]; bb[c].y += (float)q[1]; bb[c].z += (float)q[2]; bb[c].w += (float)q[3];
       }
     }
-  }
+  };
+  RowWalk w(row0, rstride, rps);
+  auto find = [&](int& fr, int& frin, int& frout, int& fsmp) {
+    for (;;) {
+      fr = w.r; fsmp = w.smp; frin = frout = -1;
+      if (fr >= R) return;
+      resolve(w, frin, frout);
+      w.next();
+      if ((frin | frout) >= 0) return;
+    }
+  };
+  int smp;
+  find(r, rin, rout, smp);
+  if (r < R) {
+    issue_x(r, rin, lane); issue_y(r, lane); issue_prev(r, lane);
+    mu = mean[rin]; rs = rstd[rin];
+    if (rowmask) km = rowmask[smp];
+  }
+  stage_columns(lg, gamma, gb, nch);
+  int r1, rin1, rout1, smp1;
+  find(r1, rin1, rout1, smp1);
+  vm_drain();
+  while (r < R) {
+    const int ol = opaque(lane);
+    reduce_row(true, ol);
+    float mu1 = 0.f, rs1 = 0.f, km1 = 1.f;
+    const bool next = r1 < R;
+    const int rl = next ? r1 : r, rinl = next ? rin1 : rin;
+    issue_x(rl, rinl, ol); issue_y(rl, ol);
+    if (next) {
+      mu1 = mean[rin1]; rs1 = rstd[rin1];
+      if (rowmask) km1 = rowmask[smp1];
+    }
+    int r2, rin2, rout2, smp2;
+    find(r2, rin2, rout2, smp2);
+    store_row(true, true, ol);
+    __builtin_amdgcn_sched_barrier(0);
+    issue_prev(rl, ol);
+    r = r1; rin = rin1; rout = rout1; mu = mu1; rs = rs1; km = km1;
+    r1 = r2; rin1 = rin2; rout1 = rout2; smp1 = smp2;
+  }
+  if (in_map || out_map) {
+    for (RowWalk v(row0, rstride, rps); v.r < R; v.next()) {
+      resolve(v, rin, rout);
+      if ((rin >= 0) == (rout >= 0)) continue;
+      r = v.r;
+      const int ol = opaque(lane);
+      issue_prev(r, ol); issue_y(r, ol);
+      mu = rs = 0.f;
+      if (rin >= 0) {
+        issue_x(r, rin, ol);
+        mu = mean[rin]; rs = rstd[rin];
+      }
+      km = rowmask ? rowmask[v.smp] : 1.f;
+      reduce_row(rin >= 0, ol);
+      store_row(rin >= 0, rout >= 0, ol);
+    }
+  }
+  __syncthreads();
   float4* r0 = reinterpret_cast<float4*>(red + (size_t)wave * 4 * D);
 #pragma unroll
   for (int c = 0; c < NCH; ++c) {
     const int i = lane + c * 64;
-    if (i < nch) { r0[i] = ag[c]; r0[nch + i] = ab[c]; r0[2 * nch + i] = HAS_Y ? bg[HAS_Y ? c : 0] : float4{0, 0, 0, 0}; r0[3 * nch + i] = bb[c]; }
+    if (chunk_ok<FULL>(i, nch)) { r0[i] = ag[c]; r0[nch + i] = ab[c]; r0[2 * nch + i] = HAS_Y ? bg[HAS_Y ? c : 0] : float4{0, 0, 0, 0}; r0[3 * nch + i] = bb[c]; }
   }
   __syncthreads();
   for (int n = threadIdx.x; n < D; n += 256) {
     float a = 0.f, b = 0.f, c2 = 0.f, d2 = 0.f;
 #pragma unroll
-    for (int w = 0; w < 4; ++w) {
-      const float* rw = red + (size_t)w * 4 * D;
+    for (int w2 = 0; w2 < 4; ++w2) {
+      const float* rw = red + (size_t)w2 * 4 * D;
       a += rw[n]; b += rw[D + n]; c2 += rw[2 * D + n]; d2 += rw[3 * D + n];
     }
     atomicAdd(dgamma + n, a);
@@ -590,6 +805,29 @@
 
 }
 
+#define ROW_DISPATCH(D, L)                                                                               \
+  do {                                                                                                   \
+    const int nchl_ = cdiv((D) / 4, 64);                                                                 \
+    const bool full_ = (D) % 256 == 0;                                                                   \
+    if (nchl_ <= 1) { if (full_) L(1, true); else L(1, false); }                                         \
+    else if (nchl_ <= 2) { if (full_) L(2, true); else L(2, false); }                                    \
+    else if (nchl_ <= 3) { if (full_) L(3, true); else L(3, false); }                                    \
+    else if (nchl_ <= 4) { if (full_) L(4, true); else L(4, false); }                                    \
+    else if (nchl_ == 5 && full_) L(5, true);                                                            \
+    else if (nchl_ == 8 && full_) L(8, true);                                                            \
+    else L(8, false);                                                                                    \
+  } while (0)
+
+#define ROW_DISPATCH4(D, L)                                                                              \
+  do {                                                                                                   \
+    const int nchl_ = cdiv((D) / 4, 64);                                                                 \
+    const bool full_ = (D) % 256 == 0;                                                                   \
+    if (nchl_ <= 1) { if (full_) L(1, true); else L(1, false); }                                         \
+    else if (nchl_ <= 2) { if (full_) L(2, true); else L(2, false); }                                    \
+    else if (nchl_ <= 3) { if (full_) L(3, true); else L(3, false); }                                    \
+    else { if (full_) L(4, true); else L(4, false); }                                                    \
+  } while (0)
+
 extern "C" int memhip_layernorm_fwd(const float* x, int64_t ldx, const int32_t* row_idx, int R, int D,
                                     const float* gamma, const float* beta, float eps, void* y,
                                     int64_t ldy, float* mean, float* rstd, memhip_stream_t stream) {
@@ -597,8 +835,11 @@
   if (R == 0) return MEMHIP_OK;
   MEMHIP_REQUIRE(x && gamma && beta && y && mean && rstd, "layernorm_fwd: null pointer");
   MEMHIP_REQUIRE(ldx % 4 == 0 && ldy % 4 == 0, "layernorm_fwd: ld must be a multiple of 4");
-  hipLaunchKernelGGL(ln_fwd_kernel, dim3(cdiv(R, 4)), dim3(256), 0, as_stream(stream), x, (long long)ldx,
-                     row_idx, R, D, gamma, beta, eps, (__bf16*)y, (long long)ldy, mean, rstd);
+#define LNF_LAUNCH(N, F)                                                                                 \
+  hipLaunchKernelGGL((ln_fwd_kernel<N, F>), dim3(cdiv(R, 4)), dim3(256), (size_t)2 * D * sizeof(float), as_stream(stream), \
+                     x, (long long)ldx, row_idx, R, D, gamma, beta, eps, (__bf16*)y, (long long)ldy, mean, rstd)
+  ROW_DISPATCH(D, LNF_LAUNCH);
+#undef LNF_LAUNCH
   return check_launch("layernorm_fwd");
 }
 
@@ -613,17 +854,15 @@
   int grid = cdiv(R, 4);
   const int cap = opt(OPT_LN_BWD_GRID) * 4 / 3;
   if (grid > cap) grid = cap;
-#define LNB_LAUNCH(N)                                                                                    \
-  hipLaunchKernelGGL(ln_bwd_kernel<N>, dim3(grid), dim3(256), (size_t)8 * D * sizeof(float), as_stream(stream), \
+#define LNB_LAUNCH(N, F)                                                                                 \
+  if (accumulate) LNB_LAUNCH2(N, F, true); else LNB_LAUNCH2(N, F, false)
+#define LNB_LAUNCH2(N, F, A)                                                                             \
+  hipLaunchKernelGGL((ln_bwd_kernel<N, F, A>), dim3(grid), dim3(256), (size_t)8 * D * sizeof(float), as_stream(stream), \
                      (const __bf16*)dy, (long long)lddy, x, (long long)ldx, row_idx, R, D, gamma, mean, rstd, dres, \
-                     (long long)lddres, accumulate, dgamma, dbeta)
-  const int nchl = cdiv(D / 4, 64);
-  if (nchl <= 1) LNB_LAUNCH(1);
-  else if (nchl <= 2) LNB_LAUNCH(2);
-  else if (nchl <= 3) LNB_LAUNCH(3);
-  else if (nchl <= 4) LNB_LAUNCH(4);
-  else LNB_LAUNCH(8);
+                     (long long)lddres, dgamma, dbeta)
+  ROW_DISPATCH(D, LNB_LAUNCH);
 #undef LNB_LAUNCH
+#undef LNB_LAUNCH2
   return check_launch("layernorm_bwd");
 }
 
@@ -642,25 +881,23 @@
   MEMHIP_REQUIRE(D <= 64 * 4 * kBrMaxChunks, "branch_bwd: D=%d too large", D);
   int grid = cdiv(M, 4);
   if (grid > 1024) grid = 1024;
-#define BRB_LAUNCH(N)                                                                                    \
-  if (drop) BRB_LAUNCH_D(N); else                                                                        \
-  hipLaunchKernelGGL(branch_bwd_kernel<N>, dim3(grid), dim3(256), (size_t)8 * D * sizeof(float), as_stream(stream), \
+#define BRB_LAUNCH(N, F)                                                                                 \
+  if (y) BRB_LAUNCH_Y(N, F, true); else BRB_LAUNCH_Y(N, F, false)
+#define BRB_LAUNCH_Y(N, F, Y)                                                                            \
+  if (drop) BRB_LAUNCH_D(N, F, Y); else                                                                  \
+  hipLaunchKernelGGL((branch_bwd_kernel<N, F, Y>), dim3(grid), dim3(256), (size_t)8 * D * sizeof(float), as_stream(stream), \
                      dx, (long long)lddx, (const __bf16*)y, (long long)ldy, gamma, rowmask, keep_prob,    \
                      rows_per_sample > 0 ? rows_per_sample : 1, M, D, (__bf16*)dy, (long long)lddy, dgamma, dbias, \
                      (const int*)out_map)
-#define BRB_LAUNCH_D(N)                                                                                  \
-  hipLaunchKernelGGL((branch_bwd_kernel<N, DropParams>), dim3(grid), dim3(256), (size_t)8 * D * sizeof(float),  \
+#define BRB_LAUNCH_D(N, F, Y)                                                                            \
+  hipLaunchKernelGGL((branch_bwd_kernel<N, F, Y, DropParams>), dim3(grid), dim3(256), (size_t)8 * D * sizeof(float),  \
                      as_stream(stream), dx, (long long)lddx, (const __bf16*)y, (long long)ldy, gamma, rowmask, keep_prob, \
                      rows_per_sample > 0 ? rows_per_sample : 1, M, D, (__bf16*)dy, (long long)lddy, dgamma, dbias, \
                      (const int*)out_map, drop_params(*drop))
-  const int nchl = cdiv(D / 4, 64);
-  if (nchl <= 1) BRB_LAUNCH(1);
-  else if (nchl <= 2) BRB_LAUNCH(2);
-  else if (nchl <= 3) BRB_LAUNCH(3);
-  else if (nchl <= 4) BRB_LAUNCH(4);
-  else BRB_LAUNCH(8);
+  ROW_DISPATCH(D, BRB_LAUNCH);
 #undef BRB_LAUNCH
 #undef BRB_LAUNCH_D
+#undef BRB_LAUNCH_Y
   return check_launch("branch_bwd");
 }
 
@@ -744,28 +981,24 @@
   int cap = opt(OPT_LN_BWD_GRID);
   if (D > 768 && cap > 512) cap = 512;
   if (grid > cap) grid = cap;
-#define LBB_LAUNCH(N)                                                                                    \
-  if (drop) { if (y_branch) LBB_LAUNCH2D(N, true); else LBB_LAUNCH2D(N, false); }                       \
-  else if (y_branch) LBB_LAUNCH2(N, true); else LBB_LAUNCH2(N, false)
-#define LBB_LAUNCH2(N, Y)                                                                                \
-  hipLaunchKernelGGL((ln_bwd_branch_kernel<N, Y>), dim3(grid), dim3(256), (size_t)16 * D * sizeof(float), \
+#define LBB_LAUNCH(N, F)                                                                                 \
+  if (drop) { if (y_branch) LBB_LAUNCH2D(N, F, true); else LBB_LAUNCH2D(N, F, false); }                 \
+  else if (y_branch) LBB_LAUNCH2(N, F, true); else LBB_LAUNCH2(N, F, false)
+#define LBB_LAUNCH2(N, F, Y)                                                                              \
+  hipLaunchKernelGGL((ln_bwd_branch_kernel<N, F, Y>), dim3(grid), dim3(256), (size_t)16 * D * sizeof(float), \
                      as_stream(stream), (const __bf16*)dy, (long long)lddy, x, (long long)ldx, R, D, gamma, mean, \
                      rstd, dres, (long long)lddres, dgamma, dbeta, (const __bf16*)y_branch, (long long)ldyb, \
                      gamma_branch, rowmask, keep_prob, rows_per_sample > 0 ? rows_per_sample : 1,         \
                      (__bf16*)dy_branch, (long long)lddyb, dgamma_branch, dbias_branch, (const int*)in_map, \
                      (const int*)out_map)
-#define LBB_LAUNCH2D(N, Y)                                                                               \
-  hipLaunchKernelGGL((ln_bwd_branch_kernel<N, Y, DropParams>), dim3(grid), dim3(256), (size_t)16 * D * sizeof(float), \
+#define LBB_LAUNCH2D(N, F, Y)                                                                            \
+  hipLaunchKernelGGL((ln_bwd_branch_kernel<N, F, Y, DropParams>), dim3(grid), dim3(256), (size_t)16 * D * sizeof(float), \
                      as_stream(stream), (const __bf16*)dy, (long long)lddy, x, (long long)ldx, R, D, gamma, mean, \
                      rstd, dres, (long long)lddres, dgamma, dbeta, (const __bf16*)y_branch, (long long)ldyb, \
                      gamma_branch, rowmask, keep_prob, rows_per_sample > 0 ? rows_per_sample : 1,         \
                      (__bf16*)dy_branch, (long long)lddyb, dgamma_branch, dbias_branch, (const int*)in_map, \
                      (const int*)out_map, drop_params(*drop))
-  const int nchl = cdiv(D / 4, 64);
-  if (nchl <= 1) LBB_LAUNCH(1);
-  else if (nchl <= 2) LBB_LAUNCH(2);
-  else if (nchl <= 3) LBB_LAUNCH(3);
-  else LBB_LAUNCH(4);
+  ROW_DISPATCH4(D, LBB_LAUNCH);
 #undef LBB_LAUNCH
 #undef LBB_LAUNCH2
 #undef LBB_LAUNCH2D
```

Result: faster. 7683 samples/sec (median of 6 runs) (+2.2%).
